# XingqunQi-lab/EmotionGestures

Hardware: AMD Instinct MI355X
Metric: gesture clips/sec (34 frames, 43 joints) (higher is better)
Workload: dtype bf16x3; 1 GPU; TED clips: 4 s 16 kHz audio -> mel(128x124) -> CVAE sample -> generator -> 34x126 pose; global_batch=64, variant=Models_spatial_memory, parallelism=clip-sharded x1, no data-path collective, launch=hipGraph replay, 4 step(s) in flight, branch_streams=False, fold_affine=False

## Files before the change

### emotiongestures_amd/_lib.py

```python
from __future__ import annotations

import ctypes as C
import os

_HERE = os.path.dirname(os.path.abspath(__file__))
LIB_PATH = os.path.join(_HERE, "libemogest_hip.so")

EG_PREC_F32, EG_PREC_BF16X3, EG_PREC_BF16 = 0, 1, 2
PRECISIONS = {"f32": EG_PREC_F32, "fp32": EG_PREC_F32, "bf16x3": EG_PREC_BF16X3, "bf16": EG_PREC_BF16}

(PACK_RAW, PACK_LINEAR, PACK_VEC_PAD, PACK_CONV3X3, PACK_BN_SCALE, PACK_BN_SHIFT, PACK_CONV1X1, PACK_STEM,
 PACK_WN_TAP, PACK_CONV1D, PACK_POS_TABLE, PACK_LINEAR_T, PACK_LINEAR_FOLD, PACK_BIAS_FOLD, PACK_CONV1X1_BF16, PACK_WN_TAPS) = range(16)


class EgError(RuntimeError):
    pass


class EgWeightEntry(C.Structure):
    _fields_ = [("key", C.c_char * 192), ("kind", C.c_int32), ("dims", C.c_int32 * 4),
                ("offset", C.c_int64), ("numel", C.c_int64)]


class EgGeneratorConfig(C.Structure):
# ... 52 lines not shown
    "eg_generator_forward_rollout": (C.c_int, [_P, _P, _I, _I, _P, _P, _P, _P, _P, _P, _P, _P, _P, _P, _P, _P, _L, _P]),
    "eg_generator_rollout_workspace_bytes": (_L, [_P, _I, _I]),
    "eg_generator_forward_rollout_draws": (C.c_int, [_P, _P, _I, _I, _I, _P, _P, _P, _P, _P, _P, _P, _P, _P, _P, _P, _P, _L, _P]),
    "eg_generator_rollout_draws_workspace_bytes": (_L, [_P, _I, _I, _I]),
    "eg_rows_by_table": (C.c_int, [_P, _P, _P, _I, _L, _I, _P]),
    "eg_rollout_ragged_plan_ints": (_L, [_I, _L]),
    "eg_rollout_ragged_plan": (C.c_int, [_P, _I, _P, _P, _P, _P]),
    "eg_generator_forward_rollout_ragged": (C.c_int, [_P, _P, _I, _P, _P, _P, _P, _P, _P, _P, _P, _P, _P, _P, _P, _P, _P, _L, _P]),
    "eg_generator_rollout_ragged_workspace_bytes": (_L, [_P, _I, _L]),
    "eg_rollout_takes_plan_ints": (_L, [_I, _L]),
    "eg_rollout_takes_plan": (C.c_int, [_P, _I, _P, _P, _P, _P]),
    "eg_generator_forward_rollout_takes": (C.c_int, [_P, _P, _I, _I, _P, _P, _P, _P, _P, _P, _P, _P, _P, _P, _P, _P, _P, _P, _L, _P]),
    "eg_generator_rollout_takes_workspace_bytes": (_L, [_P, _I, _L, _I]),
    "eg_stream_state_bytes": (_L, [_P, _I, _I, _I]),
    "eg_stream_reset": (C.c_int, [_P, _P, _I, _I, _I, _P, _P, _P]),
    "eg_stream_push": (C.c_int, [_P, _P, _I, _I, _I, _P, _P, _P, _P]),
    "eg_generator_stream_step": (C.c_int, [_P, _P, _P, _I, _I, _I, _P, _P, _P, _P, _P, _P, _P, _P, _P, _L, _P]),
    "eg_stream_tail": (C.c_int, [_P, _P, _I, _I, _I, _P, _P]),
    "eg_generator_tap": (C.c_int, [_P, _I, _P, C.c_char_p, C.POINTER(_P), C.POINTER(_L)]),
    "eg_cvae_default_config": (C.c_int, [C.POINTER(EgCvaeConfig)]),
    "eg_cvae_create": (C.c_int, [C.POINTER(EgCvaeConfig), C.POINTER(_P)]),
    "eg_cvae_destroy": (None, [_P]),
    "eg_cvae_arena_floats": (_L, [_P]),
    "eg_cvae_num_weights": (_I, [_P]),
    "eg_cvae_weight_entry": (C.c_int, [_P, _I, C.POINTER(EgWeightEntry)]),
    "eg_cvae_workspace_bytes": (_L, [_P, _I]),
    "eg_cvae_sample": (C.c_int, [_P, _P, _I, _P, _P, _P, _P, _L, _P]),
    "eg_cvae_forward": (C.c_int, [_P, _P, _I, _P, _P, _P, _P, _P, _P, _P, _L, _P]),
    "eg_mel_tables": (C.c_int, [_P, _P, _P, _P]),
    "eg_mel_workspace_bytes": (_L, [_I, _I]),
    "eg_melspectrogram": (C.c_int, [_P, _I, _I, _P, _P, _P, _P, _P, _I, _P, _L, _P]),
    "eg_window_gather": (C.c_int, [_P, _I, _L, _I, _L, _I, _P, _P]),
    "eg_window_gather_ragged": (C.c_int, [_P, _I, _L, _P, _P, _L, _I, _P, _P]),
    "eg_resample_plan": (C.c_int, [_I, _I, C.POINTER(EgResamplePlan)]),
    "eg_resample_out_length": (_L, [_L, _I, _I]),
    "eg_resample_filter": (C.c_int, [_I, _I, _P, _P]),
    "eg_resample": (C.c_int, [_P, _I, _L, _P, _P, _I, _I, _P, _L, _P, _L, _P]),
    "eg_resample_stream_state_bytes": (_L, [_I, _I, _I]),
    "eg_resample_stream_reset": (C.c_int, [_P, _I, _I, _I, _P, _P]),
    "eg_resample_stream_push": (C.c_int, [_P, _I, _I, _I, _P, _P, _I, _P, _P, _I, _P]),
    "eg_skeleton_check": (C.c_int, [_P, _P, _P, _I]),
    "eg_skeleton_out_frames": (_L, [_L, _I, _I]),
    "eg_skeleton_tile_frames": (_I, []),
    "eg_skeleton_joints": (C.c_int, [_P, _I, _I, _P, _P, _P, _I, _P, _P, _I, _I, _P, _I, _I, _I, _P, _L, _P]),
    "eg_skeleton_dir_vec": (C.c_int, [_P, _I, _I, _P, _P, _P, _I, _P, _P, _I, _I, _P, _P, _P]),
    "eg_skeleton_rest_check": (C.c_int, [_P, _I]),
    "eg_skeleton_levels": (C.c_int, [_P, _P, _P, _I, _P, _P]),
    "eg_skeleton_rotations": (C.c_int, [_P, _I, _I, _P, _P, _P, _I, _P, _P, _P, _I, _I, _P, _I, _I, _I, _P, _L, _P]),
    "eg_articulate_check": (C.c_int, [_P, _P, _I]),
    "eg_articulate_levels": (C.c_int, [_P, _P, _I, _P]),
    "eg_articulate_tile_frames": (_I, []),
    "eg_articulate_forward": (C.c_int, [_P, _I, _I, _P, _P, _I, _P, _P, _I, _I, _P, _I, _I, _I, _I, _P, _P, _L, _P]),
    "eg_articulate_rot6d": (C.c_int, [_P, _I, _I, _I, _P, _I, _I, _P, _I, _P, _P]),
    "eg_articulate_euler": (C.c_int, [_P, _I, _I, _I, _P, _P, _P, _I, _I, _P, _I, _I, _I, _I, _P, _L, _P]),
    "eg_articulate_rot6d_euler": (C.c_int, [_P, _I, _I, _I, _P, _P, _P, _I, _I, _P, _I, _I, _P, _P]),
    "eg_angle_unwrap_workspace_bytes": (_L, [_I, _I, _I]),
    "eg_angle_unwrap": (C.c_int, [_P, _I, _I, _I, _P, _I, _I, C.c_double, _P, _L, _P]),
    "eg_smooth_design": (C.c_int, [_I, _I, _I, C.c_double, _P, _P]),
    "eg_smooth_tile_frames": (_I, []),
    "eg_smooth_tile_cols": (_I, []),
    "eg_smooth_tracks": (C.c_int, [_P, _I, _I, _I, _I, _P, _P, _P, _I, _I, _P, _P]),
    "eg_smooth_stream_state_bytes": (_L, [_I, _I, _I]),
    "eg_smooth_stream_reset": (C.c_int, [_P, _I, _I, _I, _P, _P]),
    "eg_smooth_stream_push": (C.c_int, [_P, _I, _I, _I, _I, _P, _P, _P, _P, _P]),
    "eg_smooth_stream_tail": (C.c_int, [_P, _I, _I, _I, _I, _P, _P, _P, _P]),
    "eg_beat_tables": (C.c_int, [_P, _P, _P, _P]),
    "eg_beat_workspace_bytes": (_L, [_I, _I]),
    "eg_beat_align": (C.c_int, [_P, _I, _I, _P, _I, _I, _I, _I, _I, C.c_double, _I, _P, _P, _P, _P, _P, _L, _P, _P, _P, _P, _P, _P, _P]),
    "eg_beat_tracks_meta_ints": (_L, [_I]),
    "eg_beat_tracks_meta": (C.c_int, [_P, _P, _P, _I, _I, _P]),
    "eg_beat_tracks_workspace_bytes": (_L, [_P, _P, _I, _I, _I]),
    "eg_beat_align_tracks": (C.c_int, [_P, _I, _L, _P, _P, _P, _I, _I, _I, _P, _I, _I, _P, C.c_double, _I, _P, _P, _P, _P, _P, _L, _P, _P, _P,
                                       _P, _P, _P, _P]),
    "eg_beat_tracks_scan": (C.c_int, [_P, _P, _I, _P, _P, _L, _P, _P, _P]),
    "eg_take_meta_ints": (_L, [_I]),
    "eg_take_meta": (C.c_int, [_P, _I, _P]),
    "eg_track_rows_pack": (C.c_int, [_P, _I, _I, _I, _I, _P, _P, _P, _P]),
    "eg_take_distance_workspace_bytes": (_L, [_P, _I, _I]),
    "eg_take_distance": (C.c_int, [_P, _I, _I, _I, _P, _P, _I, _P, _L, _P, _P, _P]),
    "eg_conv3x3": (C.c_int, [_P, _P, _P, _P, _P, _P, _P, _I, _I, _I, _I, _I, _I, _I, _I, _I, _P]),
    "eg_conv3x3_se": (C.c_int, [_P, _P, _P, _P, _P, _P, _P, _P, _P, _I, _I, _I, _I, _I, _I, _I, _I, _I, _P]),
    "eg_se_gate_pre": (C.c_int, [_P, _P, _I, _P, _P, _P, _P, _P, _P, _P, _P, _I, _I, _I, _I, _P]),
    "eg_se_block_fused": (C.c_int, [_P] * 19 + [_I] * 7 + [_P]),
    "eg_conv3x3_gap_tiles": (_I, [_I, _I, _I, _I, _I]),
    "eg_conv3x3_channel_split": (_I, [_I, _I, _I, _I, _I, _I, _I]),
    "eg_stem_conv": (C.c_int, [_P, _P, _P, _P, _P, _P, _I, _I, _I, _I, _P]),
    "eg_se_gate": (C.c_int, [_P, _I, _P, _P, _P, _P, _P, _I, _I, _I, _P]),
    "eg_se_residual_relu": (C.c_int, [_P, _P, _P, _P, _P, _P, _P, _I, _I, _I, _I, _I, _I, _I, _I, _P]),
    "eg_linear": (C.c_int, [_P, _I, _P, _I, _P, _P, _P, _I, _P, _I, _I, _I, _I, _I, _I, _I, _I, _P]),
    "eg_split_tiles": (C.c_int, [_P, _I, _I, _I, _P, _P]),
    "eg_linear_presplit": (C.c_int, [_P, _I, _P, _I, _P, _P, _P, _I, _P, _I, _I, _I, _I, _I, _I, _P]),
    "eg_linear_presplit_causal": (C.c_int, [_P, _I, _P, _P, _I, _P, _P, _I, _P, _I, _P, _I, _I, _I, _I, _I, _I, _I, _I, _P]),
    "eg_linear_splitk": (C.c_int, [_P, _I, _P, _I, _P, _P, _I, _I, _I, _I, _I, _I, _P, _I, _P]),
    "eg_layernorm": (C.c_int, [_P, _P, _P, _P, _I, _I, C.c_float, _P]),
    "eg_attention": (C.c_int, [_P, _I, _P, _I, _P, _I, _P, _I, _P, _I, _I, _I, _I, _I, _I, _P]),
    "eg_attention_masked": (C.c_int, [_P, _I, _P, _I, _P, _I, _P, _L, _I, _P, _I, _P, _I, _I, _I, _I, _I, _I, _P]),
    "eg_mha_workspace_bytes": (_L, [_I, _I, _I, _I, _I]),
    "eg_multi_head_attention": (C.c_int, [_P, _P, _P, _P, _P, _P, _P, _P, _P, _P, _I, _I, _I, _I, _I, _I, _P, _L, _P]),
    "eg_ffn_workspace_bytes": (_L, [_I, _I, _I]),
    "eg_positionwise_ffn": (C.c_int, [_P, _P, _P, _P, _P, _P, _P, _P, _I, _I, _I, _I, _P, _L, _P]),
    "eg_tcn_forward": (C.c_int, [_P, _P, _P, _I, _I, _I, _I, _I, _P, _L, _P]),
    "eg_add_rows": (C.c_int, [_P, _P, _P, _L, _I, _I, _P]),
    "eg_add_rows_split": (C.c_int, [_P, _P, _P, _P, _L, _I, _I, _P]),
    "eg_conv3x3_packed_floats": (_L, [_I, _I]),
    "eg_profile_enable": (C.c_int, [_I]),
    "eg_profile_disable": (C.c_int, []),
    "eg_profile_read": (_I, [_P, _P, _P, _I]),
    "eg_profile_read_workgroups": (_I, [_P, _I]),
    "eg_time_linear": (C.c_int, [_P, _P, _P, _P, _I, _I, _I, _I, _P]),
    "eg_reparameterize": (C.c_int, [_P, _P, _P, _P, _L, _P]),
    "eg_conv1d": (C.c_int, [_P, _P, _P, _P, _P, _P, _I, _I, _I, _I, _I, _I, _I, _I, _P]),
    "eg_contrastive_workspace_bytes": (C.c_int64, [_I]),
    "eg_contrastive_loss": (C.c_int, [_P, _P, _I, _I, _P, _P, _P, _P, _L, _P]),
    "eg_contrastive_backward_workspace_bytes": (_L, [_I]),
    "eg_contrastive_loss_backward": (C.c_int, [_P, _P, _I, _I, _P, _P, _P, _L, _P]),
    "eg_transpose": (C.c_int, [_P, _I, _I, _I, _P, _I, _P]),
    "eg_gemm_tn_workspace_floats": (_L, [_I, _I, _L]),
    "eg_gemm_tn": (C.c_int, [_P, _I, _P, _I, _P, _I, _I, _I, _L, _P, _L, _I, _P]),
    "eg_conv3x3_wgrad": (C.c_int, [_P, _P, _P, _I, _I, _I, _I, _I, _I, _P, _L, _P]),
    "eg_im2col3x3": (C.c_int, [_P, _P, _I, _I, _I, _I, _I, _I, _P]),
    "eg_subsample": (C.c_int, [_P, _P, _I, _I, _I, _I, _I, _I, _P]),
    "eg_conv1d_cl_forward": (C.c_int, [_P, _P, _P, _P] + [_I] * 9 + [_P]),
    "eg_conv1d_cl_backward_input": (C.c_int, [_P, _P, _P, _P] + [_I] * 9 + [_P]),
    "eg_conv1d_cl_backward_weight_workspace_floats": (_L, [_I] * 7),
    "eg_conv1d_cl_backward_weight": (C.c_int, [_P, _P, _P, _P, _P] + [_I] * 9 + [_P, _L, _P]),
    "eg_pad_cols": (C.c_int, [_P, _P, _L, _I, _I, _P]),
    "eg_colreduce_workspace_floats": (_L, [_I]),
    "eg_bn_train_forward": (C.c_int, [_P, _P, _P, _P, _P, _P, _P, _P, _L, _I, C.c_float, C.c_float, _P, _P]),
    "eg_bn_train_backward": (C.c_int, [_P, _P, _P, _P, _P, _P, _P, _P, _L, _I, _I, _P, _P]),
    "eg_bn_train_forward_gap": (C.c_int, [_P, _P, _I, _I, _P, _P, _P, _P, _P, _P, _P, _P, _L, _I, C.c_float, C.c_float, _P, _P]),
    "eg_bn_train_forward_sq": (C.c_int, [_P, _P, _P, _I, _I, _P, _P, _P, _P, _P, _P, _P, _P, _L, _I, C.c_float, C.c_float, _P, _P]),
    "eg_conv3x3_sq": (C.c_int, [_P, _P, _P, _P, _P, _P] + [_I] * 8 + [_P]),
    "eg_se_gate_train_forward": (C.c_int, [_P] * 12 + [_I, _I, _I, _P]),
    "eg_se_tail_forward": (C.c_int, [_P] * 9 + [_I, _I, _I, _P]),
    "eg_se_tail_backward_reduce": (C.c_int, [_P] * 7 + [_I, _I, _I, _P, _P]),
    "eg_se_gate_train_backward": (C.c_int, [_P] * 16 + [_I, _I, _I, _P]),
    "eg_se_tail_backward_finish": (C.c_int, [_P] * 14 + [_I, _I, _I, _P]),
    "eg_se_tail_backward_apply": (C.c_int, [_P] * 13 + [_I, _I, _I, _P]),
    "eg_colsum": (C.c_int, [_P, _P, _P, _P, _L, _I, _P, _P]),
    "eg_elementwise": (C.c_int, [_P, _P, _P, _L, _I, C.c_float, _P]),
    "eg_conv3x3_wgrad_mfma_workspace_floats": (_L, [_I, _I, _I, _I, _I]),
    "eg_conv3x3_wgrad_mfma": (C.c_int, [_P, _P, _P, _I, _I, _I, _I, _I, _P, _L, _P]),
    "eg_conv3x3_wgrad_mfma_oihw": (C.c_int, [_P, _P, _P, _I, _I, _I, _I, _I, _P, _L, _P]),
    "eg_conv3x3_wgrad_gather_mfma": (C.c_int, [_P, _P, _P, _I, _I, _I, _I, _I, _I, _P, _L, _P]),
    "eg_conv3x3_dgrad_s2": (C.c_int, [_P, _P, _P, _P, _I, _I, _I, _I, _I, _I, _P]),
    "eg_conv3x3_res_masked": (C.c_int, [_P, _P, _P, _P, _P, _I, _I, _I, _I, _I, _I, _P]),
    "eg_conv3x3_wgrad_mfma_oihw_in_affine": (C.c_int, [_P, _P, _P, _P, _P, _I, _I, _I, _I, _I, _P, _L, _P]),
    "eg_conv3x3_sq_in_affine": (C.c_int, [_P, _P, _P, _P, _P, _P, _P, _P, _I, _I, _I, _I, _I, _I, _I, _I, _P]),
    "eg_bn_train_stats_sq": (C.c_int, [_P, _P, _I, _I, _P, _P, _P, _P, _P, _P, _P, _P, _L, _I, C.c_float, C.c_float, _P, _P]),
    "eg_pack_conv3x3_device": (C.c_int, [_P, _I, _I, _I, _P, _P]),
    "eg_linear_packed_floats": (_L, [_I, _I]),
    "eg_pack_linear_device": (C.c_int, [_P, _I, _I, _I, _I, _P, _P]),
    "eg_pack_table_blocks": (_I, [_I, _I, _I, _I]),
    "eg_pack_table": (C.c_int, [_P, _I, _I, _P]),
    "eg_dropout": (C.c_int, [_P, _P, _L, C.c_float, C.c_uint32, C.c_uint64, _P]),
    "eg_dropout_dev": (C.c_int, [_P, _P, _L, C.c_float, C.c_uint32, C.c_uint64, _P, _P]),
    "eg_seg_mean": (C.c_int, [_P, _P, _I, _I, _I, C.c_float, _P, _P]),
    "eg_seg_dot": (C.c_int, [_P, _P, _P, _I, _I, _I, _P, _P]),
    "eg_se_scale": (C.c_int, [_P, _P, _P, _P, _I, _I, _I, _P]),
    "eg_layernorm_backward": (C.c_int, [_P, _P, _P, _P, _P, _I, _I, C.c_float, _P]),
    "eg_attention_train": (C.c_int, [_P, _I, _P, _I, _P, _I, _P, _I, _P, _I, _I, _I, _I, _I, C.c_float, C.c_uint32, C.c_uint64, _P, _P]),
    "eg_attention_backward_train": (C.c_int, [_P, _I, _P, _I, _P, _I, _P, _P, _I, _P, _I, _P, _I, _P, _I, _I, _I, _I, _I, _I, C.c_float, C.c_uint32,
                                              C.c_uint64, _P, _P]),
    "eg_smooth_l1": (C.c_int, [_P, _P, _P, _P, _L, C.c_float, C.c_float, _P, _P]),
    "eg_cross_entropy": (C.c_int, [_P, _P, _P, C.c_float, C.c_float, _P, _P, _I, _I, _P, _P]),
    "eg_kld": (C.c_int, [_P, _P, _P, _P, _P, _I, _I, C.c_float, _P]),
# ... 53 lines not shown
```

### emotiongestures_amd/csrc/conv.hip

```cpp
#include <type_traits>
#include "common.h"


namespace {

struct ConvArgs {
    const float* x; const float* w; const float* bias; const float* scale; const float* shift;
    float* y; float* gap;
    float* gap2 = nullptr;
    int H, W, Ho, Wo, cout, relu, nchw, tiles_x, tiles;
    const float* gate = nullptr; const float* res = nullptr; int relu2 = 0;
    const float* in_scale = nullptr; const float* in_shift = nullptr;
    int wrow = 0;
    const unsigned* res_bits = nullptr;
    const float* res_q = nullptr;
    unsigned int* dbg = nullptr;
    const float* sc_x = nullptr; const bf8* sc_whi = nullptr; const bf8* sc_wlo = nullptr; const float* sc_vec = nullptr;
    int sc_H = 0, sc_W = 0, sc_S = 2, sc_B = 0;
};
__device__ __forceinline__ f4 residual_quad(const float* __restrict__ res, const unsigned* __restrict__ bits, size_t e) {
    f4 r = *reinterpret_cast<const f4*>(res + e);
    if (bits) {
        const unsigned nb = bits[e >> 5] >> (unsigned)(e & 28);
        r[0] = (nb & 1u) ? r[0] : 0.f;
        r[1] = (nb & 2u) ? r[1] : 0.f;
        r[2] = (nb & 4u) ? r[2] : 0.f;
        r[3] = (nb & 8u) ? r[3] : 0.f;
    }
    return r;
}

template <int S, int TH> struct ConvGeom {
    static constexpr int IH = (TH - 1) * S + 3;
    static constexpr int IW = 31 * S + 3;
    static constexpr int NPIX = IH * IW;
    static constexpr int PL = (S == 1) ? ((NPIX + 15) / 16 * 16) : (NPIX | 1);
    static constexpr int MT = TH * 2 / 4;
};

template <int TH> struct ConvGeomDG2 {
    static constexpr int IH = TH + 1;
    static constexpr int IW = 33;
    static constexpr int NPIX = IH * IW;
    static constexpr int PL = (NPIX + 15) / 16 * 16;
};

template <int CIN, int NT, int S, int TH>
__global__ __launch_bounds__(256) void conv3x3_f32_kernel(ConvArgs a) {
    using G = ConvGeom<S, TH>;
    constexpr int COUTP = NT * 16, IW = G::IW, NPIX = G::NPIX, PL = G::PL, MT = G::MT;
    __shared__ f4 tile[8 * PL];

    const int tid = threadIdx.x, wave = tid >> 6, lane = tid & 63, li = lane & 15, kq = lane >> 4;
    int tile_id = blockIdx.x, b = blockIdx.y;
    {
        const int total = gridDim.x * gridDim.y;
        if ((total & 7) == 0) {
            const int lin = blockIdx.y * gridDim.x + blockIdx.x;
            const int log = (lin & 7) * (total >> 3) + (lin >> 3);
            b = log / (int)gridDim.x;
            tile_id = log - b * (int)gridDim.x;
        }
    }
    const int ty = tile_id / a.tiles_x, tx = tile_id - ty * a.tiles_x;
    const int oy0 = ty * TH, ox0 = tx * 32;
    const int iy0 = oy0 * S - 1, ix0 = ox0 * S - 1;

    int pbase[MT];
#pragma unroll
    for (int t = 0; t < MT; ++t) {
        const int id = wave * MT + t;
        pbase[t] = ((id >> 1) * S) * IW + ((id & 1) * 16 + li) * S;
    }
    f4 acc[MT][NT];
#pragma unroll
    for (int t = 0; t < MT; ++t)
#pragma unroll
        for (int n = 0; n < NT; ++n) acc[t][n] = (f4){0.f, 0.f, 0.f, 0.f};

    const f4* __restrict__ w4 = reinterpret_cast<const f4*>(a.w);
    const float* __restrict__ xb = a.x + (size_t)b * a.H * a.W * CIN;

    for (int chunk = 0; chunk < CIN / 32; ++chunk) {
        if (chunk) __syncthreads();
        for (int idx = tid; idx < ((NPIX + 7) / 8) * 64; idx += 256) {
            const int p = (idx >> 6) * 8 + (idx & 7), cq = (idx >> 3) & 7;
            if (p < NPIX) {
                const int iy = p / IW, ix = p - iy * IW;
                const int gy = iy0 + iy, gx = ix0 + ix;
                f4 v = (f4){0.f, 0.f, 0.f, 0.f};
                if (gy >= 0 && gy < a.H && gx >= 0 && gx < a.W)
                    v = *reinterpret_cast<const f4*>(xb + ((size_t)gy * a.W + gx) * CIN + chunk * 32 + cq * 4);
                tile[cq * PL + p] = v;
            }
        }
        __syncthreads();
        const f4* wp = w4 + (size_t)(chunk * 8 + kq) * COUTP + li;
#pragma unroll 1
        for (int kh = 0; kh < 3; ++kh) {
#pragma unroll
            for (int kw = 0; kw < 3; ++kw) {
                const int tap = kh * 3 + kw, toff = kh * IW + kw;
// ... 393 lines not shown
    for (int t = 0; t < MT; ++t) {
        const int id = wm * MT + t;
        const int oy = oy0 + (id >> 1), ox = ox0 + (id & 1) * 16 + li;
        pixo[t] = (oy < a.Ho && ox < a.Wo) ? oy * a.Wo + ox : -1;
    }
    const int hw = a.Ho * a.Wo;
    float* __restrict__ yb = a.y + (size_t)b * hw * a.cout;
#pragma unroll
    for (int n = 0; n < NT; ++n) {
        gsum[n] = (f4){0.f, 0.f, 0.f, 0.f};
        gsq[n] = gsum[n];
        const int co = c0 + (wn * NT + n) * 16 + kq * 4;
        const f4 bi = a.bias ? *reinterpret_cast<const f4*>(a.bias + co) : (f4){0.f, 0.f, 0.f, 0.f};
        f4 sc = a.scale ? *reinterpret_cast<const f4*>(a.scale + co) : (f4){1.f, 1.f, 1.f, 1.f};
        f4 sh = a.shift ? *reinterpret_cast<const f4*>(a.shift + co) : (f4){0.f, 0.f, 0.f, 0.f};
        if constexpr (SCC > 0) {
            const float* __restrict__ qv = a.sc_vec + ((size_t)a.sc_B + b) * a.cout + co;
            sc = *reinterpret_cast<const f4*>(qv);
            sh = *reinterpret_cast<const f4*>(qv + (size_t)a.sc_B * a.cout);
        }
        const f4 gt = (a.gate && co < a.cout) ? *reinterpret_cast<const f4*>(a.gate + (size_t)b * a.cout + co) : (f4){1.f, 1.f, 1.f, 1.f};
        const bool rb = a.res != nullptr;
        const size_t rbase = (size_t)b * hw * a.cout;
#pragma unroll
        for (int t = 0; t < MT; ++t) {
            f4 v = acc[0][t][n] + bi;
            if (a.relu) {
#pragma unroll
                for (int r = 0; r < 4; ++r) v[r] = fmaxf(v[r], 0.f);
            }
            v = v * sc + sh;
            if (a.gate) v = v * gt;
            if (rb && pixo[t] >= 0 && co < a.cout) v += residual_quad(a.res, a.res_bits, rbase + (size_t)pixo[t] * a.cout + co);
            if (a.relu2) {
#pragma unroll
                for (int r = 0; r < 4; ++r) v[r] = fmaxf(v[r], 0.f);
            }
            if (pixo[t] >= 0) {
                if (!a.nchw) {
                    if (co < a.cout) *reinterpret_cast<f4*>(yb + pixo[t] * a.cout + co) = v;
                } else {
#pragma unroll
                    for (int r = 0; r < 4; ++r)
                        if (co + r < a.cout) yb[(co + r) * hw + pixo[t]] = v[r];
                }
                gsum[n] += v;
                if (a.gap2) gsq[n] += v * v;
            }
        }
    }
    if (a.gap) {
        float* sred = reinterpret_cast<float*>(lds);
#pragma unroll
        for (int n = 0; n < NT; ++n) {
#pragma unroll
            for (int r = 0; r < 4; ++r) {
                float s = gsum[n][r];
                s = row16_sum(s);
                if (li == 0) sred[wm * COUTP + (wn * NT + n) * 16 + kq * 4 + r] = s;
                if (a.gap2) {
                    float q = gsq[n][r];
                    q = row16_sum(q);
                    if (li == 0) sred[(WM + wm) * COUTP + (wn * NT + n) * 16 + kq * 4 + r] = q;
                }
            }
        }
        wait_lgkmcnt0();
        wg_barrier();
        if (tid < (SPLIT ? COUTP : a.cout)) {
            float s = 0.f;
#pragma unroll
            for (int m = 0; m < WM; ++m) s += sred[m * COUTP + tid];
            a.gap[((size_t)b * a.tiles + tile_id) * a.cout + c0 + tid] = s;
            if (a.gap2) {
                float q = 0.f;
#pragma unroll
                for (int m = 0; m < WM; ++m) q += sred[(WM + m) * COUTP + tid];
                a.gap2[((size_t)b * a.tiles + tile_id) * a.cout + c0 + tid] = q;
            }
        }
    }
}

template <int TERMS, int TH = 4, bool STAMP = false>
__global__ __launch_bounds__(256, 2) void conv3x3_c32_persistent_kernel(ConvArgs a, const bf8* __restrict__ whi, const bf8* __restrict__ wlo,
                                                                     int total_tiles, int tiles_per_wg) {
    using G = ConvGeom<1, TH>;
    constexpr int CIN = 32, IW = G::IW, NPIX = G::NPIX, PL = G::PL, MT = TH / 2, NT = 2;
    constexpr int NIMG = (TERMS == 3) ? 2 : 1;
    constexpr int TILE = NIMG * 4 * PL, WTAP = 4 * 32, WIMG = 9 * WTAP;
    static_assert(PL - NPIX >= 8 || TH == 4, "the gap scratch of the 8-row variant lives in the planes' padding slots");
    extern __shared__ __attribute__((aligned(16))) bf8 lds[];
    bf8* tile = lds;
    bf8* wl = lds + TILE;
    float* sred_base = reinterpret_cast<float*>(lds + TILE + NIMG * WIMG);
    const int sred_pitch = (TH == 4) ? 32 : PL * 4;
    float* sred = (TH == 4) ? sred_base : reinterpret_cast<float*>(tile + NPIX);

    const int tid = threadIdx.x, wave = tid >> 6, lane = tid & 63, li = lane & 15, kq = lane >> 4;
    const int wave_u = __builtin_amdgcn_readfirstlane(wave);
    int wg = blockIdx.x;
    if ((gridDim.x & 7) == 0) wg = (blockIdx.x & 7) * (gridDim.x >> 3) + (blockIdx.x >> 3);
    const int NWG = gridDim.x;
    const int t_begin = wg, t_end = total_tiles;
    (void)tiles_per_wg;
    if (t_begin >= t_end) return;

#pragma unroll
    for (int img = 0; img < NIMG; ++img) {
        const bf8* src = img ? wlo : whi;
#pragma unroll
        for (int p = 0; p < 5; ++p) {
            const int piece = p * 4 + wave_u;
            if (piece < WIMG / 64)
                __builtin_amdgcn_global_load_lds((const __attribute__((address_space(1))) void*)(src + piece * 64 + lane),
                                                 (__attribute__((address_space(3))) void*)(wl + img * WIMG + piece * 64), 16, 0, 0);
        }
    }

    constexpr int NIT = (((NPIX + 7) / 8) * 32 + 255) / 256;
    int piy[NIT], pix[NIT], lslot[NIT];
#pragma unroll
    for (int it = 0; it < NIT; ++it) {
        const int idx = tid + it * 256;
        const int p = (idx >> 5) * 8 + (idx & 7), oc = (idx >> 3) & 3;
        piy[it] = p / IW;
        pix[it] = p - piy[it] * IW;
        lslot[it] = p < NPIX ? oc * PL + p : -1;
    }
    const int oc8 = ((tid >> 3) & 3) * 8;
    f4 isc[2] = {(f4){1.f, 1.f, 1.f, 1.f}, (f4){1.f, 1.f, 1.f, 1.f}}, ish[2] = {(f4){0.f, 0.f, 0.f, 0.f}, (f4){0.f, 0.f, 0.f, 0.f}};
    if (a.in_scale) {
        isc[0] = *reinterpret_cast<const f4*>(a.in_scale + oc8); isc[1] = *reinterpret_cast<const f4*>(a.in_scale + oc8 + 4);
        ish[0] = *reinterpret_cast<const f4*>(a.in_shift + oc8); ish[1] = *reinterpret_cast<const f4*>(a.in_shift + oc8 + 4);
    }
    f4 pv[NIT][2];
    struct Coord { int b, ty, tx; };
    const int tiles_y = a.tiles / a.tiles_x;
    const int adv_b = NWG / a.tiles, adv_r = NWG - adv_b * a.tiles, adv_ty = adv_r / a.tiles_x, adv_tx = adv_r - adv_ty * a.tiles_x;
    auto advance = [&](Coord& c) {
        c.tx += adv_tx;
        if (c.tx >= a.tiles_x) { c.tx -= a.tiles_x; ++c.ty; }
        c.ty += adv_ty;
        if (c.ty >= tiles_y) { c.ty -= tiles_y; ++c.b; }
        c.b += adv_b;
    };
    auto load_tile = [&](const Coord& c) {
        const int b = c.b;
        const int iy0 = c.ty * TH - 1, ix0 = c.tx * 32 - 1;
        const float* __restrict__ xb = a.x + (size_t)b * a.H * a.W * CIN;
#pragma unroll
        for (int it = 0; it < NIT; ++it) {
            pv[it][0] = pv[it][1] = (f4){0.f, 0.f, 0.f, 0.f};
            const int gy = iy0 + piy[it], gx = ix0 + pix[it];
            if (lslot[it] >= 0 && gy >= 0 && gy < a.H && gx >= 0 && gx < a.W) {
                const float* src = xb + (gy * a.W + gx) * CIN + oc8;
                pv[it][0] = *reinterpret_cast<const f4*>(src);
                pv[it][1] = *reinterpret_cast<const f4*>(src + 4);
                if (a.in_scale) {
                    pv[it][0] = pv[it][0] * isc[0] + ish[0];
                    pv[it][1] = pv[it][1] * isc[1] + ish[1];
                }
            }
        }
    };
    auto store_tile = [&]() {
#pragma unroll
        for (int it = 0; it < NIT; ++it) {
            if (lslot[it] >= 0) {
                bf8 hi, lo;
                split_octet<TERMS == 3>(pv[it][0], pv[it][1], hi, lo);
                tile[lslot[it]] = hi;
                if (TERMS == 3) tile[4 * PL + lslot[it]] = lo;
            }
        }
    };
    int pbase[MT];
#pragma unroll
    for (int t = 0; t < MT; ++t) {
        const int id = wave * MT + t;
        pbase[t] = (id >> 1) * IW + (id & 1) * 16 + li;
    }
    struct Frags { bf8 wh[NT], wlf[NT], xh[MT], xl[MT]; };
    auto read_frags = [&](Frags& f, int tap) {
        const bf8* Wh = wl + tap * WTAP + kq * 32 + li;
        const int kh = tap / 3, kw = tap - kh * 3, toff = kh * IW + kw;
#pragma unroll
        for (int n = 0; n < NT; ++n) {
            f.wh[n] = Wh[n * 16];
            if (TERMS == 3) f.wlf[n] = Wh[WIMG + n * 16];
        }
#pragma unroll
        for (int t = 0; t < MT; ++t) {
            f.xh[t] = tile[kq * PL + pbase[t] + toff];
            if (TERMS == 3) f.xl[t] = tile[(4 + kq) * PL + pbase[t] + toff];
        }
    };

    const int hw = a.Ho * a.Wo;
    f4 bi[NT], sc[NT], sh[NT];
#pragma unroll
    for (int n = 0; n < NT; ++n) {
        const int co = n * 16 + kq * 4;
        bi[n] = a.bias ? *reinterpret_cast<const f4*>(a.bias + co) : (f4){0.f, 0.f, 0.f, 0.f};
        sc[n] = a.scale ? *reinterpret_cast<const f4*>(a.scale + co) : (f4){1.f, 1.f, 1.f, 1.f};
        sh[n] = a.shift ? *reinterpret_cast<const f4*>(a.shift + co) : (f4){0.f, 0.f, 0.f, 0.f};
    }

    f4 rsn[MT][NT];
    auto load_res = [&](const Coord& c) {
        const int ty = c.ty, tx = c.tx;
        const size_t rbase = (size_t)c.b * hw * 32;
#pragma unroll
        for (int t = 0; t < MT; ++t) {
            const int id = wave * MT + t;
            const int oy = ty * TH + (id >> 1), ox = tx * 32 + (id & 1) * 16 + li;
            const bool ok = a.res && oy < a.Ho && ox < a.Wo;
#pragma unroll
            for (int n = 0; n < NT; ++n)
                rsn[t][n] = ok ? residual_quad(a.res, a.res_bits, rbase + (size_t)(oy * a.Wo + ox) * 32 + n * 16 + kq * 4) : (f4){0.f, 0.f, 0.f, 0.f};
        }
    };
    Coord cur;
    cur.b = t_begin / a.tiles;
    cur.ty = (t_begin - cur.b * a.tiles) / a.tiles_x;
    cur.tx = t_begin - cur.b * a.tiles - cur.ty * a.tiles_x;
    Coord nxt = cur;
    load_tile(cur);
    load_res(cur);
    wait_vmcnt_imm<0>();
    unsigned int ph[6] = {0, 0, 0, 0, 0, 0};
    unsigned long long tk = 0;
    auto stamp = [&](int i) {
        if constexpr (STAMP) {
            const unsigned long long now = __builtin_amdgcn_s_memtime();
            if (i >= 0) ph[i] += (unsigned int)(now - tk);
            tk = now;
        }
    };
    for (int L = t_begin; L < t_end; L += NWG, cur = nxt) {
        const int b = cur.b, tile_id = cur.ty * a.tiles_x + cur.tx;
        const int oy0 = cur.ty * TH, ox0 = cur.tx * 32;
        advance(nxt);
        stamp(-1);
        store_tile();
        stamp(0);
        __syncthreads();
        stamp(1);
        int pixo[MT];
        f4 rs[MT][NT];
#pragma unroll
        for (int t = 0; t < MT; ++t) {
            const int id = wave * MT + t;
            const int oy = oy0 + (id >> 1), ox = ox0 + (id & 1) * 16 + li;
            pixo[t] = (oy < a.Ho && ox < a.Wo) ? oy * a.Wo + ox : -1;
#pragma unroll
            for (int n = 0; n < NT; ++n) rs[t][n] = rsn[t][n];
        }
        const bool has_res = a.res != nullptr;
        if (L + NWG < t_end) load_res(nxt);
        if (L + NWG < t_end) load_tile(nxt);
        stamp(2);

        f4 acc[MT][NT];
#pragma unroll
        for (int t = 0; t < MT; ++t)
#pragma unroll
            for (int n = 0; n < NT; ++n) acc[t][n] = (f4){0.f, 0.f, 0.f, 0.f};
        Frags fr[2];
        read_frags(fr[0], 0);
#pragma unroll
        for (int tap = 0; tap < 9; ++tap) {
            if (tap < 8) read_frags(fr[(tap + 1) & 1], tap + 1);
            const Frags& f = fr[tap & 1];
#pragma unroll
            for (int t = 0; t < MT; ++t)
#pragma unroll
                for (int n = 0; n < NT; ++n) {
                    if (TERMS == 3) {
                        acc[t][n] = __builtin_amdgcn_mfma_f32_16x16x32_bf16(f.wlf[n], f.xh[t], acc[t][n], 0, 0, 0);
                        acc[t][n] = __builtin_amdgcn_mfma_f32_16x16x32_bf16(f.wh[n], f.xl[t], acc[t][n], 0, 0, 0);
                    }
                    acc[t][n] = __builtin_amdgcn_mfma_f32_16x16x32_bf16(f.wh[n], f.xh[t], acc[t][n], 0, 0, 0);
                }
        }

        if constexpr (STAMP) {
#pragma unroll
            for (int t = 0; t < MT; ++t)
#pragma unroll
                for (int n = 0; n < NT; ++n) asm volatile("" : "+v"(acc[t][n]));
        }
        stamp(3);
        float* __restrict__ yb = a.y + (size_t)b * hw * 32;
        f4 gsum[NT], gsq[NT];
#pragma unroll
        for (int n = 0; n < NT; ++n) {
            gsum[n] = (f4){0.f, 0.f, 0.f, 0.f};
            gsq[n] = gsum[n];
            const int co = n * 16 + kq * 4;
            const f4 gt = a.gate ? *reinterpret_cast<const f4*>(a.gate + (size_t)b * 32 + co) : (f4){1.f, 1.f, 1.f, 1.f};
#pragma unroll
            for (int t = 0; t < MT; ++t) {
                f4 v = acc[t][n] + bi[n];
                if (a.relu) {
#pragma unroll
                    for (int r = 0; r < 4; ++r) v[r] = fmaxf(v[r], 0.f);
                }
                v = v * sc[n] + sh[n];
                if (a.gate) v = v * gt;
                if (has_res && pixo[t] >= 0) v += rs[t][n];
                if (a.relu2) {
#pragma unroll
                    for (int r = 0; r < 4; ++r) v[r] = fmaxf(v[r], 0.f);
                }
                if (pixo[t] >= 0) {
                    *reinterpret_cast<f4*>(yb + pixo[t] * 32 + co) = v;
                    gsum[n] += v;
                    if (a.gap2) gsq[n] += v * v;
                }
            }
        }
        if (a.gap) {
#pragma unroll
            for (int n = 0; n < NT; ++n)
#pragma unroll
                for (int r = 0; r < 4; ++r) {
                    float sm = gsum[n][r];
                    sm = row16_sum(sm);
                    if (li == 0) sred[wave * sred_pitch + n * 16 + kq * 4 + r] = sm;
                    if (a.gap2) {
                        float q = gsq[n][r];
                        q = row16_sum(q);
                        if (li == 0) sred[128 + wave * 32 + n * 16 + kq * 4 + r] = q;
                    }
                }
        }
        stamp(4);
        __syncthreads();
        stamp(5);
        if (a.gap && tid < 32) {
            float sm = 0.f;
#pragma unroll
            for (int m = 0; m < 4; ++m) sm += sred[m * sred_pitch + tid];
            a.gap[((size_t)b * a.tiles + tile_id) * 32 + tid] = sm;
            if (a.gap2) a.gap2[((size_t)b * a.tiles + tile_id) * 32 + tid] = (sred[128 + tid] + sred[160 + tid]) + (sred[192 + tid] + sred[224 + tid]);
        }
    }
    if constexpr (STAMP) {
        if (lane == 0 && a.dbg)
#pragma unroll
            for (int i = 0; i < 6; ++i) a.dbg[((size_t)blockIdx.x * 4 + wave) * 8 + i] = ph[i];
    }
}

__global__ __launch_bounds__(256) void stem_conv_kernel(const float* __restrict__ x, const float* __restrict__ w,
                                                        const float* __restrict__ bias, const float* __restrict__ scale,
                                                        const float* __restrict__ shift, float* __restrict__ y,
                                                        int B, int H, int W, int C) {
    extern __shared__ float rows[];
    const int cq_n = C >> 2, tid = threadIdx.x;
    const int b = blockIdx.x / H, oy = blockIdx.x - b * H, WP = W + 2;
    const float* xb = x + (size_t)b * H * W;
    for (int i = tid; i < 3 * WP; i += 256) {
        const int r = i / WP, c = i - r * WP, gy = oy + r - 1, gx = c - 1;
        rows[i] = (gy >= 0 && gy < H && gx >= 0 && gx < W) ? xb[gy * W + gx] : 0.f;
    }
    const int cq = tid % cq_n, px0 = tid / cq_n, pstep = 256 / cq_n;
    f4 wv[9];
#pragma unroll
    for (int t = 0; t < 9; ++t) wv[t] = *reinterpret_cast<const f4*>(w + t * C + cq * 4);
    const f4 bi = *reinterpret_cast<const f4*>(bias + cq * 4);
    const f4 sc = *reinterpret_cast<const f4*>(scale + cq * 4), sh = *reinterpret_cast<const f4*>(shift + cq * 4);
    __syncthreads();
    float* yrow = y + ((size_t)b * H + oy) * W * C + cq * 4;
    for (int ox = px0; ox < W; ox += pstep) {
        f4 acc = bi;
#pragma unroll
        for (int kh = 0; kh < 3; ++kh)
#pragma unroll
            for (int kw = 0; kw < 3; ++kw) acc += wv[kh * 3 + kw] * rows[kh * WP + ox + kw];
#pragma unroll
        for (int r = 0; r < 4; ++r) acc[r] = fmaxf(acc[r], 0.f);
        *reinterpret_cast<f4*>(yrow + (size_t)ox * C) = acc * sc + sh;
    }
}

__global__ __launch_bounds__(256) void se_gate_kernel(const float* __restrict__ gap, int tiles, const float* __restrict__ w1,
                                                      const float* __restrict__ b1, const float* __restrict__ w2,
                                                      const float* __restrict__ b2, float* __restrict__ gate, int C, float inv_hw) {
    __shared__ float m[256];
    __shared__ float h[32];
    const int b = blockIdx.x, t = threadIdx.x, R = C >> 3;
    {
        const int c = t % C, g = t / C, G = blockDim.x / C;
        float s = 0.f;
        for (int i = g; i < tiles; i += G) s += gap[((size_t)b * tiles + i) * C + c];
        m[t] = s;
        __syncthreads();
        float tot = 0.f;
        if (t < C)
            for (int j = 0; j < G; ++j) tot += m[j * C + t];
        __syncthreads();
        if (t < C) m[t] = tot * inv_hw;
    }
    __syncthreads();
    if (t < R) {
        float s = b1[t];
        for (int c = 0; c < C; ++c) s += w1[t * C + c] * m[c];
        h[t] = fmaxf(s, 0.f);
    }
    __syncthreads();
    if (t < C) {
        float s = b2[t];
        for (int j = 0; j < R; ++j) s += w2[t * R + j] * h[j];
        gate[(size_t)b * C + t] = 1.f / (1.f + expf(-s));
    }
}

constexpr int GP_T = 1024;
__global__ __launch_bounds__(GP_T) void se_gate_pre_kernel(const float* __restrict__ t1, const float* __restrict__ gap, int tiles,
                                                           const float* __restrict__ w2img, const float* __restrict__ scale2,
                                                           const float* __restrict__ shift2, const float* __restrict__ w1, const float* __restrict__ b1,
                                                           const float* __restrict__ wf2, const float* __restrict__ bf2, float* __restrict__ gate,
                                                           int H, int W, int C, const float* __restrict__ ds_scale, const float* __restrict__ ds_shift,
                                                           float* __restrict__ sc_vec) {
    extern __shared__ __attribute__((aligned(16))) float sm[];
    const int b = blockIdx.x, t = threadIdx.x, G = GP_T / C, c = t % C, g = t / C, R = C >> 3;
    float* part = sm;
    float* S = sm + 5 * GP_T;
    float* zp = S + 9 * C;
    float* m = zp + GP_T;
    float* hbuf = m + C;
    const float* tb = t1 + (size_t)b * H * W * C;
    float s0 = 0.f, s1 = 0.f, s2 = 0.f, s3 = 0.f, s4 = 0.f;
#pragma unroll 4
    for (int i = g; i < tiles; i += G) s0 += gap[((size_t)b * tiles + i) * C + c];
#pragma unroll 4
    for (int x = g; x < W; x += G) {
        s1 += tb[(size_t)x * C + c];
        s2 += tb[((size_t)(H - 1) * W + x) * C + c];
    }
#pragma unroll 4
    for (int y = g; y < H; y += G) {
        s3 += tb[((size_t)y * W) * C + c];
        s4 += tb[((size_t)y * W + W - 1) * C + c];
    }
    part[t] = s0; part[GP_T + t] = s1; part[2 * GP_T + t] = s2; part[3 * GP_T + t] = s3; part[4 * GP_T + t] = s4;
    __syncthreads();
    if (t < C) {
        float T = 0.f, R0 = 0.f, RL = 0.f, C0 = 0.f, CL = 0.f;
        for (int j = 0; j < G; ++j) {
            T += part[j * C + t]; R0 += part[GP_T + j * C + t]; RL += part[2 * GP_T + j * C + t]; C0 += part[3 * GP_T + j * C + t];
            CL += part[4 * GP_T + j * C + t];
        }
        const float c00 = tb[t], c0L = tb[(size_t)(W - 1) * C + t], cL0 = tb[((size_t)(H - 1) * W) * C + t], cLL = tb[((size_t)(H - 1) * W + W - 1) * C + t];
#pragma unroll
        for (int kh = 0; kh < 3; ++kh)
#pragma unroll
            for (int kw = 0; kw < 3; ++kw) {
                const float rex = kh == 0 ? RL : (kh == 2 ? R0 : 0.f);
                const float cex = kw == 0 ? CL : (kw == 2 ? C0 : 0.f);
                float corner = 0.f;
                if (kh == 0 && kw == 0) corner = cLL;
                if (kh == 0 && kw == 2) corner = cL0;
                if (kh == 2 && kw == 0) corner = c0L;
                if (kh == 2 && kw == 2) corner = c00;
// ... 86 lines not shown
        }
        const f4 res = acc * *reinterpret_cast<const f4*>(dss + cq * 4) + *reinterpret_cast<const f4*>(dsh + cq * 4);
        const f4 g = *reinterpret_cast<const f4*>(gate + (size_t)b * COUT + cq * 4);
        f4 v = *reinterpret_cast<const f4*>(y + p * COUT + cq * 4) * g + res;
#pragma unroll
        for (int r = 0; r < 4; ++r) v[r] = fmaxf(v[r], 0.f);
        *reinterpret_cast<f4*>(out + p * COUT + cq * 4) = v;
      }
    }
}

template <int CIN, int NT, int S, int TH, int WM, int WN, int TERMS, int SCC = 0>
int launch_conv_bf16(const ConvArgs& a, const bf8* whi, const bf8* wlo, dim3 grid, hipStream_t st) {
    constexpr int RING = 3;
    using G = ConvGeom<S, TH>;
    constexpr int NIMG = (TERMS == 3) ? 2 : 1;
    constexpr size_t LDS_BYTES = sizeof(bf8) * (size_t)(NIMG * 4 * G::PL + RING * NIMG * 4 * NT * 16);
    auto kern = conv3x3_bf16_kernel<CIN, NT, S, TH, WM, WN, TERMS, RING, false, false, SCC>;
    if (int rc = eg_ensure_dynamic_lds(reinterpret_cast<const void*>(kern), LDS_BYTES, "conv3x3")) return rc;
    hipLaunchKernelGGL(kern, grid, dim3(256), LDS_BYTES, st, a, whi, wlo);
    return eg_check_launch("conv3x3");
}

template <int CIN, int NTS, int TH, int WM, int WN, int TERMS, int SCC = 0>
int launch_conv_split_t(ConvArgs a, int batch, const bf8* whi, const bf8* wlo, hipStream_t st) {
    constexpr int RING = 3;
    using G = ConvGeom<1, TH>;
    constexpr int NIMG = (TERMS == 3) ? 2 : 1;
    constexpr size_t LDS_BYTES = sizeof(bf8) * (size_t)(NIMG * 4 * G::PL + RING * NIMG * 4 * NTS * 16);
    auto kern = conv3x3_bf16_kernel<CIN, NTS, 1, TH, WM, WN, TERMS, RING, true, false, SCC>;
    if (int rc = eg_ensure_dynamic_lds(reinterpret_cast<const void*>(kern), LDS_BYTES, "conv3x3 (channel split)")) return rc;
    a.wrow = a.cout;
    hipLaunchKernelGGL(kern, dim3(a.tiles, batch, a.cout / (NTS * 16)), dim3(256), LDS_BYTES, st, a, whi, wlo);
    return eg_check_launch("conv3x3 (channel split)");
}
template <int KCH, int NTN, int TH, int WM, int WN>
int launch_dgrad_s2_t(const ConvArgs& a, int batch, const bf8* whi, const bf8* wlo, hipStream_t st) {
    constexpr int RING = 3;
    using G = ConvGeomDG2<TH>;
    constexpr size_t LDS_BYTES = sizeof(bf8) * (size_t)(2 * 4 * G::PL + RING * 2 * 4 * NTN * 16);
    auto kern = conv3x3_bf16_kernel<KCH, NTN, 1, TH, WM, WN, 3, RING, false, true>;
    if (int rc = eg_ensure_dynamic_lds(reinterpret_cast<const void*>(kern), LDS_BYTES, "conv3x3 (stride-2 input gradient)")) return rc;
    dim3 grid(eg_cdiv(a.W, 32) * eg_cdiv(a.H, TH), batch);
    hipLaunchKernelGGL(kern, grid, dim3(256), LDS_BYTES, st, a, whi, wlo);
    return eg_check_launch("conv3x3 (stride-2 input gradient)");
}
int conv_channel_split(int wgs, int max_split) {
    const char* e = getenv("EG_CONV_SPLIT");
    const int forced = (e && e[0]) ? atoi(e) : -1;
    if (forced >= 0) return (forced == 2 || forced == 4) && forced <= max_split ? forced : 1;
    int split = 1;
    while (split < max_split && wgs * split * 2 <= 512) split *= 2;
    return split;
}

int body_channel_split(int batch, int tiles, int cin, int cout, int stride, int precision, int nchw_out) {
    if (!((cin == 64 || cin == 128) && cout == cin && stride == 1 && precision == EG_PREC_BF16X3 && !nchw_out)) return 1;
    return conv_channel_split(tiles * batch, cin == 128 ? 4 : 2);
}

template <int CIN, int NT, int S, int TH, int WM, int WN, int SCC = 0>
int launch_conv(const ConvArgs& a, int batch, int precision, hipStream_t st) {
    dim3 grid(a.tiles, batch), block(256);
    if (precision == EG_PREC_F32) {
        if constexpr (SCC > 0) {
            eg_set_error("conv3x3: the fused downsample shortcut exists in the split-bf16 modes only");
            return EG_ERR_UNSUPPORTED;
        }
        hipLaunchKernelGGL((conv3x3_f32_kernel<CIN, NT, S, TH>), grid, block, 0, st, a);
        return eg_check_launch("conv3x3");
    }
    const size_t f32_floats = (size_t)9 * CIN * NT * 16;
    const bf8* whi = reinterpret_cast<const bf8*>(a.w + f32_floats);
    const bf8* wlo = whi + (size_t)9 * (CIN / 8) * NT * 16;
    if (precision == EG_PREC_BF16X3) return launch_conv_bf16<CIN, NT, S, TH, WM, WN, 3, SCC>(a, whi, wlo, grid, st);
    return launch_conv_bf16<CIN, NT, S, TH, WM, WN, 1, SCC>(a, whi, wlo, grid, st);
}

bool conv32_persistent_enabled() {
    static const bool on = [] { const char* e = getenv("EG_CONV32_PERSISTENT"); return !(e && e[0] == '0'); }();
    return on;
}

template <int TERMS, int TH>
int launch_conv32_persistent_t(const ConvArgs& a, int batch, const bf8* whi, const bf8* wlo, hipStream_t st) {
    using G = ConvGeom<1, TH>;
    constexpr int NIMG = (TERMS == 3) ? 2 : 1;
    constexpr size_t LDS_BYTES = sizeof(bf8) * (size_t)(NIMG * 4 * G::PL + NIMG * 9 * 128) + (TH == 4 ? 2 * 4 * 32 * sizeof(float) : 0);
    auto kern = conv3x3_c32_persistent_kernel<TERMS, TH>;
    if (int rc = eg_ensure_dynamic_lds(reinterpret_cast<const void*>(kern), LDS_BYTES, "conv3x3 (32 -> 32, persistent)")) return rc;
    const int total = a.tiles * batch;
    const int cap = 512;
    int grid = total < cap ? total : cap;
    int tpw = eg_cdiv(total, grid);
    grid = eg_cdiv(total, tpw);
    if (grid >= 8) grid = (int)eg_round_up(grid, 8);
    hipLaunchKernelGGL(kern, dim3(grid), dim3(256), LDS_BYTES, st, a, whi, wlo, total, tpw);
    return eg_check_launch("conv3x3 (32 -> 32, persistent)");
}
int launch_conv32_persistent(const ConvArgs& a, int batch, int precision, int th, hipStream_t st) {
    const size_t f32_floats = (size_t)9 * 32 * 32;
    const bf8* whi = reinterpret_cast<const bf8*>(a.w + f32_floats);
    const bf8* wlo = whi + (size_t)9 * 4 * 32;
    static const bool stamp = [] { const char* e = getenv("EG_CONV32_STAMP"); return e && e[0] == '1'; }();
    if (stamp && precision == EG_PREC_BF16X3 && th == 4) {
        static unsigned int* dbg = nullptr;
        const int nwords = 512 * 4 * 8;
        if (!dbg && hipMalloc(&dbg, nwords * sizeof(unsigned int)) != hipSuccess) return EG_ERR_HIP;
        (void)hipMemsetAsync(dbg, 0, nwords * sizeof(unsigned int), st);
        ConvArgs b = a;
        b.dbg = dbg;
        constexpr size_t LDS_BYTES = sizeof(bf8) * (size_t)(2 * 4 * ConvGeom<1, 4>::PL + 2 * 9 * 128) + 2 * 4 * 32 * sizeof(float);
        auto kern = conv3x3_c32_persistent_kernel<3, 4, true>;
        if (int rc = eg_ensure_dynamic_lds(reinterpret_cast<const void*>(kern), LDS_BYTES, "conv3x3 (stamps)")) return rc;
        const int total = a.tiles * batch;
        int grid = total < 512 ? total : 512;
        grid = eg_cdiv(total, eg_cdiv(total, grid));
        if (grid >= 8) grid = (int)eg_round_up(grid, 8);
        hipLaunchKernelGGL(kern, dim3(grid), dim3(256), LDS_BYTES, st, b, whi, wlo, total, 0);
        static unsigned int host[512 * 4 * 8];
        if (hipMemcpyAsync(host, dbg, sizeof(host), hipMemcpyDeviceToHost, st) != hipSuccess || hipStreamSynchronize(st) != hipSuccess) return EG_ERR_HIP;
        double sum[6] = {0, 0, 0, 0, 0, 0};
        int nw = 0;
        for (int w = 0; w < grid * 4; ++w) {
            if (host[w * 8 + 3] == 0) continue;
            ++nw;
            for (int i = 0; i < 6; ++i) sum[i] += host[w * 8 + i];
        }
        const double tiles_per_wave = (double)total / grid;
        fprintf(stderr, "conv32 stamps (cycles per tile and wave, %d waves, %s residual): store_tile %.0f  barrier1 %.0f  issue_loads %.0f  taps %.0f  epilogue %.0f  barrier2 %.0f\n",
                nw, a.res ? "with" : "no", sum[0] / nw / tiles_per_wave, sum[1] / nw / tiles_per_wave, sum[2] / nw / tiles_per_wave, sum[3] / nw / tiles_per_wave,
                sum[4] / nw / tiles_per_wave, sum[5] / nw / tiles_per_wave);
        return eg_check_launch("conv3x3 (32 -> 32, stamps)");
    }
    if (th == 8) {
        if (precision == EG_PREC_BF16X3) return launch_conv32_persistent_t<3, 8>(a, batch, whi, wlo, st);
        return launch_conv32_persistent_t<1, 8>(a, batch, whi, wlo, st);
    }
    if (precision == EG_PREC_BF16X3) return launch_conv32_persistent_t<3, 4>(a, batch, whi, wlo, st);
    return launch_conv32_persistent_t<1, 4>(a, batch, whi, wlo, st);
}

int conv_tile_rows(int cin, int cout, int stride) {
    if (stride == 2 || cout >= 256) return 2;
    if (cin == 32 && cout == 32) {
        static const int th = [] { const char* e = getenv("EG_CONV32_TH"); return (e && atoi(e) == 8) ? 8 : 4; }();
        return th;
    }
    return (cout >= 128 || cin >= 128) ? 4 : 8;
}

}

extern "C" int32_t eg_conv3x3_gap_tiles(int32_t h, int32_t wdt, int32_t cin, int32_t cout, int32_t stride) {
    const int ho = (h + 2 - 3) / stride + 1, wo = (wdt + 2 - 3) / stride + 1;
    const int th = conv_tile_rows(cin, cout, stride);
    return eg_cdiv(ho, th) * eg_cdiv(wo, 32);
}

extern "C" int32_t eg_conv3x3_channel_split(int32_t batch, int32_t h, int32_t wdt, int32_t cin, int32_t cout, int32_t stride, int32_t precision) {
    return body_channel_split(batch, eg_conv3x3_gap_tiles(h, wdt, cin, cout, stride), cin, cout, stride, precision, 0);
}

extern "C" int64_t eg_conv3x3_packed_floats(int32_t cin, int32_t cout_pad) {
    return (int64_t)9 * cin * cout_pad * 2;
}

extern "C" int eg_conv3x3(const float* x, const float* w, const float* bias, const float* scale, const float* shift,
                          float* y, float* gap_partial, int32_t batch, int32_t h, int32_t wdt, int32_t cin, int32_t cout,
                          int32_t stride, int32_t relu, int32_t nchw_out, int32_t precision, void* stream) {
    return eg_conv3x3_se(x, w, bias, scale, shift, nullptr, nullptr, y, gap_partial, batch, h, wdt, cin, cout, stride, relu, nchw_out, precision, stream);
}

namespace {
struct ShortcutArgs { const float* x; const float* wimg; const float* vec; int h, w, cin, stride; };
int conv3x3_dispatch(const float* x, const float* w, const float* bias, const float* scale, const float* shift, const float* gate, const float* residual,
                     float* y, float* gap_partial, float* gap_sq, int32_t batch, int32_t h, int32_t wdt, int32_t cin, int32_t cout, int32_t stride,
                     int32_t relu, int32_t nchw_out, int32_t precision, void* stream, const float* in_scale = nullptr, const float* in_shift = nullptr,
                     const uint32_t* res_bits = nullptr, const ShortcutArgs* sc = nullptr);
}
extern "C" int eg_conv3x3_se(const float* x, const float* w, const float* bias, const float* scale, const float* shift, const float* gate,
                             const float* residual, float* y, float* gap_partial, int32_t batch, int32_t h, int32_t wdt, int32_t cin,
                             int32_t cout, int32_t stride, int32_t relu, int32_t nchw_out, int32_t precision, void* stream) {
    return conv3x3_dispatch(x, w, bias, scale, shift, gate, residual, y, gap_partial, nullptr, batch, h, wdt, cin, cout, stride, relu, nchw_out, precision, stream);
}
extern "C" int eg_conv3x3_res_masked(const float* x, const float* w, const float* residual, const uint32_t* res_bits, float* y, int32_t batch, int32_t h,
                                     int32_t wdt, int32_t cin, int32_t cout, int32_t precision, void* stream) {
    EG_REQUIRE(residual && res_bits, EG_ERR_BAD_ARG, "eg_conv3x3_res_masked: the residual and its bit mask are required");
    return conv3x3_dispatch(x, w, nullptr, nullptr, nullptr, nullptr, residual, y, nullptr, nullptr, batch, h, wdt, cin, cout, 1, 0, 0, precision, stream, nullptr,
                            nullptr, res_bits);
}
extern "C" int eg_conv3x3_sq(const float* x, const float* w, const float* bias, float* y, float* gap_partial, float* gap_sq_partial, int32_t batch, int32_t h,
                             int32_t wdt, int32_t cin, int32_t cout, int32_t stride, int32_t relu, int32_t precision, void* stream) {
    EG_REQUIRE(gap_partial && gap_sq_partial, EG_ERR_BAD_ARG, "eg_conv3x3_sq: both partial buffers are required");
    EG_REQUIRE(precision != EG_PREC_F32, EG_ERR_UNSUPPORTED, "eg_conv3x3_sq: split-bf16 modes only (the fp32 kernel emits sums only)");
    EG_REQUIRE(!(cin == 32 && cout == 32 && stride == 1) || conv_tile_rows(cin, cout, stride) == 4, EG_ERR_UNSUPPORTED,
               "eg_conv3x3_sq: the 8-row experiment tiles of the 32 -> 32 kernel have no room for the squares scratch");
    return conv3x3_dispatch(x, w, bias, nullptr, nullptr, nullptr, nullptr, y, gap_partial, gap_sq_partial, batch, h, wdt, cin, cout, stride, relu, 0, precision,
                            stream);
}
extern "C" int eg_conv3x3_sq_in_affine(const float* x, const float* in_scale, const float* in_shift, const float* w, const float* bias, float* y,
                                       float* gap_partial, float* gap_sq_partial, int32_t batch, int32_t h, int32_t wdt, int32_t cin, int32_t cout,
                                       int32_t stride, int32_t relu, int32_t precision, void* stream) {
    EG_REQUIRE(in_scale && in_shift, EG_ERR_BAD_ARG, "eg_conv3x3_sq_in_affine: both affine vectors are required");
    EG_REQUIRE(!gap_partial == !gap_sq_partial, EG_ERR_BAD_ARG, "eg_conv3x3_sq_in_affine: both partial buffers or none");
    return conv3x3_dispatch(x, w, bias, nullptr, nullptr, nullptr, nullptr, y, gap_partial, gap_sq_partial, batch, h, wdt, cin, cout, stride, relu, 0, precision,
                            stream, in_scale, in_shift);
}
namespace {
int conv3x3_dispatch(const float* x, const float* w, const float* bias, const float* scale, const float* shift, const float* gate, const float* residual,
                     float* y, float* gap_partial, float* gap_sq, int32_t batch, int32_t h, int32_t wdt, int32_t cin, int32_t cout, int32_t stride,
                     int32_t relu, int32_t nchw_out, int32_t precision, void* stream, const float* in_scale, const float* in_shift, const uint32_t* res_bits,
                     const ShortcutArgs* sc) {
    EG_REQUIRE(x && w && y && batch > 0 && h > 0 && wdt > 0, EG_ERR_BAD_ARG, "eg_conv3x3: null pointer or empty shape");
    EG_REQUIRE(!res_bits || (residual && !gate && ((size_t)batch * h * wdt * cout) % 32 == 0), EG_ERR_BAD_ARG,
               "eg_conv3x3_res_masked: the bit mask needs a residual, no gate and a map of a multiple of 32 elements");
    EG_REQUIRE((in_scale == nullptr) == (in_shift == nullptr) && (!in_scale || (precision != EG_PREC_F32 && cin % 32 == 0 && eg_aligned16(in_scale) &&
               eg_aligned16(in_shift))), EG_ERR_BAD_ARG, "eg_conv3x3: the input affine needs both vectors, a split-bf16 mode and cin %% 32 == 0");
    EG_REQUIRE(!gate || residual, EG_ERR_BAD_ARG, "eg_conv3x3_se: a gate needs a residual");
    EG_REQUIRE(!residual || (!nchw_out && stride == 1 && cout % 4 == 0 && (!gate || eg_aligned16(gate)) && eg_aligned16(residual) && residual != y),
               EG_ERR_BAD_ARG, "eg_conv3x3_se: the fused residual needs NHWC output, stride 1, cout %% 4 == 0 and a residual buffer distinct from y");
    EG_REQUIRE(eg_aligned16(x) && eg_aligned16(w) && eg_aligned16(y), EG_ERR_ALIGN, "eg_conv3x3: pointers must be 16-byte aligned");
    EG_REQUIRE(stride == 1 || stride == 2, EG_ERR_UNSUPPORTED, "eg_conv3x3: stride %d", stride);
    EG_REQUIRE(precision >= 0 && precision <= 2, EG_ERR_BAD_ARG, "eg_conv3x3: precision %d", precision);
    EG_REQUIRE(nchw_out || (cout % 4 == 0), EG_ERR_UNSUPPORTED, "eg_conv3x3: NHWC output needs cout %% 4 == 0");
    ConvArgs a;
    a.x = x; a.w = w; a.bias = bias; a.scale = scale; a.shift = shift; a.y = y; a.gap = gap_partial; a.gap2 = gap_sq;
    a.gate = gate; a.res = residual; a.relu2 = gate ? 1 : 0;
    a.res_bits = res_bits;
    a.in_scale = in_scale; a.in_shift = in_shift;
    a.H = h; a.W = wdt; a.Ho = (h + 2 - 3) / stride + 1; a.Wo = (wdt + 2 - 3) / stride + 1;
    a.cout = cout; a.relu = relu; a.nchw = nchw_out;
    const int th = conv_tile_rows(cin, cout, stride);
    a.tiles_x = eg_cdiv(a.Wo, 32);
    a.tiles = a.tiles_x * eg_cdiv(a.Ho, th);
    hipStream_t st = (hipStream_t)stream;
    const int coutp = (int)eg_round_up(cout, 16);
    EgProfScope prof((int64_t)cin * 1000000 + (int64_t)cout * 1000 + stride * 100 + 1,
                     2.0 * 9 * cin * cout * (double)a.Ho * a.Wo * batch, st);
    if (sc) {
        EG_REQUIRE(precision != EG_PREC_F32 && stride == 1 && !nchw_out && cout == cin && (cin == 64 || cin == 128) && sc->cin * 2 == cin, EG_ERR_UNSUPPORTED,
                   "conv3x3: the fused downsample shortcut serves 32 -> 64 and 64 -> 128 block entries in the split-bf16 modes (cin=%d cout=%d shortcut cin=%d)",
                   cin, cout, sc->cin);
        EG_REQUIRE(sc->x && sc->wimg && sc->vec && !gate && !residual && !bias && !relu && !gap_sq && !in_scale && sc->stride >= 1 &&
                   (sc->h - 1) / sc->stride + 1 == h && (sc->w - 1) / sc->stride + 1 == wdt && eg_aligned16(sc->x) && eg_aligned16(sc->wimg) &&
                   eg_aligned16(sc->vec), EG_ERR_BAD_ARG, "conv3x3: fused downsample shortcut: null / misaligned operand or a block input that does not map onto the output");
        a.sc_x = sc->x; a.sc_vec = sc->vec; a.sc_H = sc->h; a.sc_W = sc->w; a.sc_S = sc->stride; a.sc_B = batch;
        a.sc_whi = reinterpret_cast<const bf8*>(sc->wimg);
        a.sc_wlo = a.sc_whi + (size_t)(sc->cin / 8) * cout;
        a.scale = a.shift = nullptr;
        a.relu2 = 1;
        const int split = body_channel_split(batch, a.tiles, cin, cout, 1, precision, 0);
        const bf8* whi = reinterpret_cast<const bf8*>(a.w + (size_t)9 * cin * cout);
        const bf8* wlo = whi + (size_t)9 * (cin / 8) * cout;
        if (cin == 64 && split == 2) return launch_conv_split_t<64, 2, 8, 4, 1, 3, 1>(a, batch, whi, wlo, st);
        if (cin == 64) return launch_conv<64, 4, 1, 8, 4, 1, 1>(a, batch, precision, st);
        if (split == 2) return launch_conv_split_t<128, 4, 4, 2, 2, 3, 2>(a, batch, whi, wlo, st);
        if (split == 4) return launch_conv_split_t<128, 2, 4, 2, 2, 3, 2>(a, batch, whi, wlo, st);
        return launch_conv<128, 8, 1, 4, 2, 2, 2>(a, batch, precision, st);
    }
    if (cin == 32 && coutp == 32 && cout == 32 && stride == 1 && precision != EG_PREC_F32 && !nchw_out && conv32_persistent_enabled())
        return launch_conv32_persistent(a, batch, precision, th, st);
    if (cin == 32 && coutp == 32 && stride == 1 && th == 4) return launch_conv<32, 2, 1, 4, 4, 1>(a, batch, precision, st);
    if (cin == 32 && coutp == 32 && stride == 1) return launch_conv<32, 2, 1, 8, 4, 1>(a, batch, precision, st);
    if (cin == 32 && coutp == 64 && stride == 2) return launch_conv<32, 4, 2, 2, 2, 2>(a, batch, precision, st);
    if (const int split = body_channel_split(batch, a.tiles, cin, cout, stride, precision, nchw_out); split > 1) {
        const size_t f32_floats = (size_t)9 * cin * cout;
        const bf8* whi = reinterpret_cast<const bf8*>(a.w + f32_floats);
        const bf8* wlo = whi + (size_t)9 * (cin / 8) * cout;
        if (cin == 64 && split == 2) return launch_conv_split_t<64, 2, 8, 4, 1, 3>(a, batch, whi, wlo, st);
        if (cin == 128 && split == 2) return launch_conv_split_t<128, 4, 4, 2, 2, 3>(a, batch, whi, wlo, st);
        if (cin == 128 && split == 4) return launch_conv_split_t<128, 2, 4, 2, 2, 3>(a, batch, whi, wlo, st);
    }
    if (cin == 64 && coutp == 64 && stride == 1) return launch_conv<64, 4, 1, 8, 4, 1>(a, batch, precision, st);
    if (cin == 64 && coutp == 128 && stride == 2) return launch_conv<64, 8, 2, 2, 2, 2>(a, batch, precision, st);
    if (cin == 64 && coutp == 128 && stride == 1) return launch_conv<64, 8, 1, 4, 2, 2>(a, batch, precision, st);
    if (cin == 128 && coutp == 128 && stride == 1) return launch_conv<128, 8, 1, 4, 2, 2>(a, batch, precision, st);
    if (cin == 128 && coutp == 256 && stride == 2) return launch_conv<128, 16, 2, 2, 1, 4>(a, batch, precision, st);
    if (cin == 256 && coutp == 256 && stride == 1) return launch_conv<256, 16, 1, 2, 1, 4>(a, batch, precision, st);
    if (cin == 128 && coutp <= 64 && stride == 1) {
        if (coutp <= 48) return launch_conv<128, 3, 1, 4, 4, 1>(a, batch, precision, st);
        return launch_conv<128, 4, 1, 4, 4, 1>(a, batch, precision, st);
    }
    if (cin == 128 && coutp <= 128 && stride == 1) return launch_conv<128, 8, 1, 4, 2, 2>(a, batch, precision, st);
    eg_set_error("eg_conv3x3: unsupported channels cin=%d cout=%d stride=%d", cin, cout, stride);
    return EG_ERR_UNSUPPORTED;
}
}

extern "C" int eg_conv3x3_dgrad_s2(const float* dy, const float* w_flip, const float* res_q, float* dx, int32_t batch, int32_t h, int32_t wdt, int32_t cin,
                                   int32_t cout, int32_t precision, void* stream) {
    EG_REQUIRE(dy && w_flip && dx && batch > 0 && h > 0 && wdt > 0, EG_ERR_BAD_ARG, "eg_conv3x3_dgrad_s2: null pointer or empty shape");
    EG_REQUIRE(precision == EG_PREC_BF16X3, EG_ERR_UNSUPPORTED, "eg_conv3x3_dgrad_s2: split-bf16 arithmetic only (precision %d)", precision);
    EG_REQUIRE(eg_aligned16(dy) && eg_aligned16(w_flip) && eg_aligned16(dx) && (!res_q || eg_aligned16(res_q)), EG_ERR_ALIGN,
               "eg_conv3x3_dgrad_s2: pointers must be 16-byte aligned");
    ConvArgs a;
    a.x = dy; a.w = w_flip; a.bias = nullptr; a.scale = nullptr; a.shift = nullptr; a.y = dx; a.gap = nullptr;
    a.H = (h - 1) / 2 + 1; a.W = (wdt - 1) / 2 + 1; a.Ho = h; a.Wo = wdt;
    a.cout = cin; a.relu = 0; a.nchw = 0; a.tiles_x = eg_cdiv(a.W, 32); a.tiles = 0;
    a.res_q = res_q;
    hipStream_t st = (hipStream_t)stream;
    const size_t f32_floats = (size_t)9 * cout * cin;
    const bf8* whi = reinterpret_cast<const bf8*>(w_flip + f32_floats);
    const bf8* wlo = whi + (size_t)9 * (cout / 8) * cin;
    EgProfScope prof((int64_t)cin * 1000000 + (int64_t)cout * 1000 + 200 + 8, 2.0 * 9 * cin * cout * (double)a.H * a.W * batch, st);
    if (cin == 32 && cout == 64) return launch_dgrad_s2_t<64, 2, 4, 4, 1>(a, batch, whi, wlo, st);
    if (cin == 64 && cout == 128) return launch_dgrad_s2_t<128, 4, 2, 2, 2>(a, batch, whi, wlo, st);
    if (cin == 128 && cout == 256) return launch_dgrad_s2_t<256, 8, 1, 1, 4>(a, batch, whi, wlo, st);
    eg_set_error("eg_conv3x3_dgrad_s2: unsupported channels %d -> %d", cin, cout);
    return EG_ERR_UNSUPPORTED;
}

extern "C" int eg_stem_conv(const float* x, const float* w9xc, const float* bias, const float* scale, const float* shift,
                            float* y, int32_t batch, int32_t h, int32_t wdt, int32_t c, void* stream) {
    EG_REQUIRE(x && w9xc && bias && scale && shift && y && batch > 0, EG_ERR_BAD_ARG, "eg_stem_conv: null pointer");
    EG_REQUIRE(c % 4 == 0 && c <= 128 && 256 % (c / 4) == 0, EG_ERR_UNSUPPORTED, "eg_stem_conv: C=%d", c);
    hipLaunchKernelGGL(stem_conv_kernel, dim3(batch * h), dim3(256), 3 * (wdt + 2) * sizeof(float), (hipStream_t)stream, x, w9xc, bias, scale, shift, y,
                       batch, h, wdt, c);
    return eg_check_launch("stem_conv");
}

extern "C" int eg_se_gate(const float* gap_partial, int32_t tiles, const float* w1, const float* b1, const float* w2,
                          const float* b2, float* gate, int32_t batch, int32_t c, int32_t hw, void* stream) {
    EG_REQUIRE(gap_partial && w1 && b1 && w2 && b2 && gate && batch > 0, EG_ERR_BAD_ARG, "eg_se_gate: null pointer");
    EG_REQUIRE(c % 8 == 0 && c <= 256 && (c <= 128 ? 128 % c : 256 % c) == 0, EG_ERR_UNSUPPORTED, "eg_se_gate: C=%d", c);
    hipLaunchKernelGGL(se_gate_kernel, dim3(batch), dim3(c <= 128 ? 128 : 256), 0, (hipStream_t)stream, gap_partial, tiles, w1, b1, w2, b2,
                       gate, c, 1.0f / (float)hw);
    return eg_check_launch("se_gate");
}

namespace {
int se_gate_pre_launch(const float* t1, const float* gap_partial, int32_t tiles, const float* conv2_w, const float* scale2,
                       const float* shift2, const float* w1, const float* b1, const float* w2, const float* b2, float* gate,
                       int32_t batch, int32_t h, int32_t wdt, int32_t c, void* stream, const float* ds_scale, const float* ds_shift, float* sc_vec) {
    EG_REQUIRE(t1 && gap_partial && conv2_w && scale2 && shift2 && w1 && b1 && w2 && b2 && gate && batch > 0 && h > 1 && wdt > 1, EG_ERR_BAD_ARG,
               "eg_se_gate_pre: null pointer or empty shape");
    EG_REQUIRE(c % 8 == 0 && c <= 256 && 256 % c == 0 && eg_aligned16(conv2_w), EG_ERR_UNSUPPORTED, "eg_se_gate_pre: C=%d", c);
    const size_t smem = sizeof(float) * (5 * GP_T + 9 * (size_t)c + GP_T + c + (c >> 3) + 4);
    EG_REQUIRE(!sc_vec || (ds_scale && ds_shift), EG_ERR_BAD_ARG, "eg_se_gate_pre: the shortcut vectors need the downsample BatchNorm");
    hipLaunchKernelGGL(se_gate_pre_kernel, dim3(batch), dim3(GP_T), smem, (hipStream_t)stream, t1, gap_partial, tiles, conv2_w, scale2, shift2, w1,
                       b1, w2, b2, gate, h, wdt, c, ds_scale, ds_shift, sc_vec);
    return eg_check_launch("se_gate_pre");
}
}

extern "C" int eg_se_gate_pre(const float* t1, const float* gap_partial, int32_t tiles, const float* conv2_w, const float* scale2,
                              const float* shift2, const float* w1, const float* b1, const float* w2, const float* b2, float* gate,
                              int32_t batch, int32_t h, int32_t wdt, int32_t c, void* stream) {
    return se_gate_pre_launch(t1, gap_partial, tiles, conv2_w, scale2, shift2, w1, b1, w2, b2, gate, batch, h, wdt, c, stream, nullptr, nullptr, nullptr);
}

extern "C" int eg_se_block_fused(const float* x, const float* conv1_w, const float* scale1, const float* shift1, const float* conv2_w, const float* scale2,
                                 const float* shift2, const float* se_w1, const float* se_b1, const float* se_w2, const float* se_b2, const float* ds_w,
                                 const float* ds_scale, const float* ds_shift, float* t1, float* out, float* gap_partial, float* gate, float* sc_vec,
                                 int32_t batch, int32_t h, int32_t wdt, int32_t cin, int32_t cout, int32_t stride, int32_t precision, void* stream) {
    EG_REQUIRE(x && conv1_w && scale1 && shift1 && conv2_w && scale2 && shift2 && t1 && out && gap_partial && gate, EG_ERR_BAD_ARG, "eg_se_block_fused: null pointer");
    EG_REQUIRE(ds_w ? (ds_scale && ds_shift && sc_vec) : (cin == cout && stride == 1), EG_ERR_BAD_ARG,
               "eg_se_block_fused: a downsample needs its BatchNorm and the shortcut vectors; an identity shortcut needs cin == cout and stride 1");
    EG_REQUIRE(stride == 1 || stride == 2, EG_ERR_UNSUPPORTED, "eg_se_block_fused: stride %d", stride);
    const int ho = (h + 2 - 3) / stride + 1, wo = (wdt + 2 - 3) / stride + 1;
    if (int rc = eg_conv3x3(x, conv1_w, nullptr, scale1, shift1, t1, gap_partial, batch, h, wdt, cin, cout, stride, 1, 0, precision, stream)) return rc;
    const int tiles1 = eg_conv3x3_gap_tiles(h, wdt, cin, cout, stride);
    if (int rc = se_gate_pre_launch(t1, gap_partial, tiles1, conv2_w, scale2, shift2, se_w1, se_b1, se_w2, se_b2, gate, batch, ho, wo, cout, stream,
                                    ds_w ? ds_scale : nullptr, ds_w ? ds_shift : nullptr, ds_w ? sc_vec : nullptr)) return rc;
    if (!ds_w) return eg_conv3x3_se(t1, conv2_w, nullptr, scale2, shift2, gate, x, out, nullptr, batch, ho, wo, cout, cout, 1, 0, 0, precision, stream);
    const ShortcutArgs sc{x, ds_w, sc_vec, h, wdt, cin, stride};
    return conv3x3_dispatch(t1, conv2_w, nullptr, nullptr, nullptr, nullptr, nullptr, out, nullptr, nullptr, batch, ho, wo, cout, cout, 1, 0, 0, precision, stream,
                            nullptr, nullptr, nullptr, &sc);
}

extern "C" int eg_se_residual_relu(const float* y, const float* gate, const float* x_in, const float* ds_w,
                                   const float* ds_scale, const float* ds_shift, float* out, int32_t batch, int32_t ho,
                                   int32_t wo, int32_t c, int32_t h_in, int32_t w_in, int32_t cin, int32_t stride, void* stream) {
    EG_REQUIRE(y && gate && x_in && out && batch > 0, EG_ERR_BAD_ARG, "eg_se_residual_relu: null pointer");
    hipStream_t st = (hipStream_t)stream;
    if (!ds_w) {
        EG_REQUIRE(cin == c && h_in == ho && w_in == wo, EG_ERR_BAD_ARG, "eg_se_residual_relu: identity shortcut shape mismatch");
        const size_t n4 = (size_t)batch * ho * wo * c / 4;
        const int blocks = (int)((n4 + 255) / 256 < 8192 ? (n4 + 255) / 256 : 8192);
        hipLaunchKernelGGL(se_tail_identity_kernel, dim3(blocks), dim3(256), 0, st, reinterpret_cast<const f4*>(y), gate,
                           reinterpret_cast<const f4*>(x_in), reinterpret_cast<f4*>(out), n4, ho * wo * (c / 4), c / 4);
        return eg_check_launch("se_tail");
    }
    EG_REQUIRE(ds_scale && ds_shift, EG_ERR_BAD_ARG, "eg_se_residual_relu: downsample BN missing");
    const size_t total = (size_t)batch * ho * wo * (c / 4);
    const int blocks = (int)((total + 255) / 256 < 4096 ? (total + 255) / 256 : 4096);
    if (cin == 32 && c == 64)
        hipLaunchKernelGGL((se_tail_downsample_kernel<32, 64>), dim3(blocks), dim3(256), 32 * 64 * 4, st, y, gate, x_in, ds_w, ds_scale,
                           ds_shift, out, batch, ho, wo, h_in, w_in, stride);
    else if (cin == 64 && c == 128)
        hipLaunchKernelGGL((se_tail_downsample_kernel<64, 128>), dim3(blocks), dim3(256), 64 * 128 * 4, st, y, gate, x_in, ds_w, ds_scale,
                           ds_shift, out, batch, ho, wo, h_in, w_in, stride);
    else if (cin == 128 && c == 256) {
        if (int rc = eg_ensure_dynamic_lds(reinterpret_cast<const void*>(se_tail_downsample_kernel<128, 256>), 128 * 256 * 4, "eg_se_residual_relu")) return rc;
        hipLaunchKernelGGL((se_tail_downsample_kernel<128, 256>), dim3(blocks < 1024 ? blocks : 1024), dim3(256), 128 * 256 * 4, st, y, gate,
                           x_in, ds_w, ds_scale, ds_shift, out, batch, ho, wo, h_in, w_in, stride);
    } else {
        eg_set_error("eg_se_residual_relu: unsupported downsample %d->%d", cin, c);
        return EG_ERR_UNSUPPORTED;
    }
    return eg_check_launch("se_tail_downsample");
}
```

### emotiongestures_amd/csrc/generator.hip

```cpp
#include "common.h"
#include <string>
#include <vector>
#include <algorithm>
#include <string.h>
#include <map>
#include <mutex>

static thread_local char g_err[512] = "";
void eg_set_error(const char* fmt, ...) {
    va_list ap;
    va_start(ap, fmt);
    vsnprintf(g_err, sizeof(g_err), fmt, ap);
    va_end(ap);
}
extern "C" const char* eg_last_error(void) { return g_err; }
std::atomic<long long> g_eg_launches{0};
extern "C" int64_t eg_launch_count(void) { return (int64_t)g_eg_launches.load(std::memory_order_relaxed); }
bool g_eg_launch_hist = [] { const char* e = getenv("EG_LAUNCH_HIST"); return e && e[0] == '1'; }();
namespace {
std::mutex g_hist_mu;
std::map<std::string, long long> g_hist;
}
void egi_count_launch(const char* what) {
    std::lock_guard<std::mutex> lk(g_hist_mu);
// ... 179 lines not shown
}
void add_bn(Layout& L, const std::string& prefix, int n, int npad, int64_t& scale, int64_t& shift) {
    scale = L.add(prefix, EG_PACK_BN_SCALE, n, npad, 0, 0, npad);
    shift = L.add(prefix, EG_PACK_BN_SHIFT, n, npad, 0, 0, npad);
}
LinW add_linear_cat(Layout& L, const std::vector<std::string>& prefixes, int n_each, int k, bool bias) {
    LinW w;
    const int n = n_each * (int)prefixes.size();
    w.n = n; w.k = k; w.npad = (int)eg_round_up(n, 64); w.kpad = (int)eg_round_up(k, 64);
    std::string wk, bk;
    for (size_t i = 0; i < prefixes.size(); ++i) {
        wk += (i ? "|" : "") + prefixes[i] + ".weight";
        bk += (i ? "|" : "") + prefixes[i] + ".bias";
    }
    w.w = L.add(wk, EG_PACK_LINEAR, n, k, w.npad, w.kpad, (int64_t)w.npad * w.kpad * 2);
    if (bias) w.b = L.vec(bk, n, w.npad);
    return w;
}
LinW add_linear_fold(Layout& L, const std::string& chains, int n, int k, int kpad_force = 0, int npad_force = 0) {
    LinW w;
    w.n = n; w.k = k;
    w.npad = npad_force ? npad_force : (int)eg_round_up(n, 64);
    w.kpad = kpad_force ? kpad_force : (int)eg_round_up(k, 64);
    w.w = L.add(chains, EG_PACK_LINEAR_FOLD, n, k, w.npad, w.kpad, (int64_t)w.npad * w.kpad * 2);
    w.b = L.add(chains, EG_PACK_BIAS_FOLD, n, w.npad, 0, 0, w.npad);
    return w;
}
MhaW add_mha(Layout& L, const std::string& p, int d, bool self_attn) {
    MhaW m;
    if (self_attn) {
        m.qkv = add_linear_cat(L, {p + ".w_qs", p + ".w_ks", p + ".w_vs"}, d, d, false);
    } else {
        m.q = add_linear(L, p + ".w_qs", d, d, false);
        m.kv = add_linear_cat(L, {p + ".w_ks", p + ".w_vs"}, d, d, false);
    }
    m.o = add_linear(L, p + ".fc", d, d, false);
    m.ln_g = L.raw(p + ".layer_norm.weight", d);
    m.ln_b = L.raw(p + ".layer_norm.bias", d);
    return m;
}
FfnW add_ffn(Layout& L, const std::string& p, int d, int di) {
    FfnW f;
    f.w1 = add_linear(L, p + ".w_1", di, d, true);
    f.w2 = add_linear(L, p + ".w_2", d, di, true);
    f.ln_g = L.raw(p + ".layer_norm.weight", d);
    f.ln_b = L.raw(p + ".layer_norm.bias", d);
    return f;
}

struct Carver {
    int64_t off = 0;
    int64_t take(int64_t floats) {
        const int64_t o = off;
        off = eg_round_up(off + floats * (int64_t)sizeof(float), 256);
        return o;
    }
};

}

struct EgGenerator {
    EgGeneratorConfig cfg;
    Layout L;
    int H1, W1, H2, W2, H3, W3, HW3, Dpad, stages[3] = {3, 4, 6}, filters[3] = {32, 64, 128};
    int64_t stem_w, stem_b, stem_scale, stem_shift;
    std::vector<BlockW> blocks;
    ConvW final_conv;
    LinW a_fc1, a_fc2, emosem0, emo2, sem2, fus0, fus2, cls[4], post[4], prior_h0, prior_h2, txt_dec;
    bool fuse_se = true;
    bool fold = false;
    bool shared_chip = false;
    LinW f_audio, f_emo, f_sem, f_post, f_prior;
    int64_t pos_table;
    std::vector<MhaW> enc_attn, dec_attn;
    std::vector<FfnW> enc_ffn, dec_ffn;
    int64_t pc_w1, pc_b1, pc_s1, pc_t1, pc_w2, pc_b2, pc_s2, pc_t2;
    int64_t sp_w0, sp_b0, sp_w1, sp_b1, tc_w0, tc_b0, tc_w1, tc_b1, tm_w0, tm_b0, tm_w1, tm_b1;
    int64_t emb;
    struct TcnConv { LinW tap0, tap1, taps; int64_t bias; };
    std::vector<TcnConv> tcn;
    int64_t txt_fc1_w, txt_fc1_b;
    int Cpad;
    bool keep_taps = false;
    bool concurrent = false;
    mutable hipStream_t side[2] = {nullptr, nullptr};
    mutable hipEvent_t ev_fork = nullptr, ev_join[2] = {nullptr, nullptr};
    int ensure_streams() const {
        if (side[0]) return EG_OK;
        for (int i = 0; i < 2; ++i) {
            if (hipStreamCreateWithFlags(&side[i], hipStreamNonBlocking) != hipSuccess ||
                hipEventCreateWithFlags(&ev_join[i], hipEventDisableTiming) != hipSuccess) {
                eg_set_error("cannot create side stream/event");
                return EG_ERR_HIP;
            }
        }
        if (hipEventCreateWithFlags(&ev_fork, hipEventDisableTiming) != hipSuccess) { eg_set_error("cannot create event"); return EG_ERR_HIP; }
        return EG_OK;
    }
    ~EgGenerator() {
        for (int i = 0; i < 2; ++i) {
            if (side[i]) (void)hipStreamDestroy(side[i]);
            if (ev_join[i]) (void)hipEventDestroy(ev_join[i]);
        }
        if (ev_fork) (void)hipEventDestroy(ev_fork);
    }
};

namespace {

struct GenWs {
    int64_t act[3], gap, gate, scv, amap, afc1, afeat, emo_t, emo, sem_t, sem, cls_part, cls_h[3], cls_out;
    int64_t fus_in, fus_h, fusion, xa, xb, q, qkv, ao, proj, ffn_h, im_x[2], im_enc, im_h, im_a[3], im_p[2];
    int64_t prior_cat, prior_h, prior_enc, prior_rep, tm_mem, tm_pe, tm_gram, post_a, post_b, post_c, pose;
    int64_t t_emb, t_a, t_b, t_c, t_out, im_t[3], t_zero;
    int64_t tap_stem, tap_l[3];
    int64_t total;
};

GenWs carve(const EgGenerator* g, int B, int NB = 0) {
    if (NB <= 0) NB = B;
    const EgGeneratorConfig& c = g->cfg;
    GenWs w;
    Carver cv;
    const int64_t BF = (int64_t)B * c.frames, D = c.d_model, NF = (int64_t)NB * c.frames;
    const int64_t act = (int64_t)B * g->H1 * g->W1 * 32;
    for (int i = 0; i < 3; ++i) w.act[i] = cv.take(act);
    {
        int64_t gap_per_clip = 0;
        int h = g->H1, wd = g->W1;
        for (const BlockW& b : g->blocks) {
            const int ho = (h + 2 - 3) / b.stride + 1, wo = (wd + 2 - 3) / b.stride + 1;
            const int64_t need = (int64_t)eg_conv3x3_gap_tiles(ho, wo, b.cout, b.cout, 1) * b.cout;
            gap_per_clip = need > gap_per_clip ? need : gap_per_clip;
            const int64_t need1 = (int64_t)eg_conv3x3_gap_tiles(h, wd, b.cin, b.cout, b.stride) * b.cout;
            gap_per_clip = need1 > gap_per_clip ? need1 : gap_per_clip;
            h = ho; wd = wo;
        }
        w.gap = cv.take((int64_t)B * gap_per_clip);
    }
    w.gate = cv.take((int64_t)B * 128);
    w.scv = cv.take((int64_t)3 * B * 128);
    w.amap = cv.take(BF * g->HW3);
    w.afc1 = cv.take(BF * D); w.afeat = cv.take(BF * D);
    w.emo_t = cv.take(BF * D * 2); w.emo = cv.take(BF * D); w.sem_t = cv.take(16); w.sem = cv.take(BF * D);
    w.cls_part = cv.take((int64_t)(c.frames > 64 ? c.frames : 64) * B * D);
    w.cls_h[0] = cv.take((int64_t)B * D); w.cls_h[1] = cv.take((int64_t)B * 256); w.cls_h[2] = cv.take((int64_t)B * 64);
    w.cls_out = cv.take((int64_t)B * 16);
    w.fus_in = cv.take(NF * D); w.fus_h = cv.take(NF * D); w.fusion = cv.take(NF * D);
    w.xa = cv.take(NF * D); w.xb = cv.take(NF * D);
    w.q = cv.take(NF * D); w.qkv = cv.take(NF * D * 3); w.ao = cv.take(NF * D); w.proj = cv.take(NF * D);
    w.ffn_h = cv.take(NF * c.d_inner);
    {
        const int64_t N64 = eg_round_up(NF, 64), B64 = eg_round_up(BF, 64), KX = D > g->Dpad ? D : g->Dpad;
        w.im_x[0] = cv.take(N64 * KX); w.im_x[1] = cv.take(N64 * KX); w.im_enc = cv.take(N64 * D); w.im_h = cv.take(N64 * c.d_inner);
        w.im_a[0] = cv.take(B64 * D); w.im_a[1] = cv.take(B64 * D); w.im_a[2] = cv.take(B64 * D * 2);
        w.im_p[0] = cv.take(B64 * D); w.im_p[1] = cv.take(B64 * D);
    }
    w.prior_cat = cv.take(BF * g->Dpad); w.prior_h = cv.take(BF * D); w.prior_enc = cv.take(BF * D);
    w.prior_rep = cv.take(NB > B ? NF * D : 16);
    w.tm_mem = cv.take((int64_t)B * c.pose_dim); w.tm_pe = cv.take((int64_t)B * c.chunk + 16); w.tm_gram = cv.take((int64_t)c.pose_dim * c.chunk);
    w.post_a = cv.take(NF * D * 4); w.post_b = cv.take(NF * D); w.post_c = cv.take(NF * g->Dpad); w.pose = cv.take(NF * c.pose_dim);
    const int64_t BT = (int64_t)B * c.text_len;
    w.t_emb = cv.take(BT * g->Cpad); w.t_a = cv.take(BT * g->Cpad); w.t_b = cv.take(BT * g->Cpad); w.t_c = cv.take(BT * g->Cpad);
    w.t_out = cv.take(BT * 512);
    for (int i = 0; i < 3; ++i) w.im_t[i] = cv.take(eg_round_up(BT, 64) * g->Cpad);
    w.t_zero = cv.take((int64_t)g->Cpad * 32);
// ... 10 lines not shown

inline float* P(void* ws, int64_t off) { return reinterpret_cast<float*>(reinterpret_cast<char*>(ws) + off); }

int run_linear(const float* arena, const LinW& w, const float* x, int lda, float* y, int ldc, int m, int relu, const float* res1,
               int ldr, int prec, hipStream_t st, int n_override = 0) {
    return eg_linear(x, lda, arena + w.w, w.kpad, w.b >= 0 ? arena + w.b : nullptr, res1, nullptr, ldr, y, ldc, m,
                     n_override ? n_override : w.n, w.kpad <= lda ? w.kpad : w.k, relu, 0, 0, prec, st);
}

int run_conv(const float* arena, const ConvW& c, const float* x, float* y, float* gap, int B, int h, int w, int relu, int nchw,
             int prec, hipStream_t st) {
    return eg_conv3x3(x, arena + c.w, c.bias >= 0 ? arena + c.bias : nullptr, c.scale >= 0 ? arena + c.scale : nullptr,
                      c.shift >= 0 ? arena + c.shift : nullptr, y, gap, B, h, w, c.cin, c.cout, c.stride, relu, nchw, prec, st);
}

struct Act { float* f = nullptr; int ld = 0; void* img = nullptr; int kimg = 0; };
inline Act act(float* f, int ld, void* img = nullptr, int kimg = 0) { Act a; a.f = f; a.ld = ld; a.img = img; a.kimg = kimg; return a; }

int lin(const EgGenerator* g, const float* arena, const LinW& w, const Act& x, int xk0, const Act& y, bool want_f32, int m, int relu,
        const float* res1, int ldr, hipStream_t st, int n_override = 0, int splits = 0, float* partial = nullptr) {
    const bool img_ok = g->cfg.precision != EG_PREC_F32;
    EgiLinear p;
    p.w = arena + w.w; p.ldw = w.kpad; p.bias = w.b >= 0 ? arena + w.b : nullptr;
    p.res1 = res1; p.ldr = ldr; p.m = m; p.n = n_override ? n_override : w.n; p.relu = relu; p.precision = g->cfg.precision;
    p.shared_chip = g->shared_chip ? 1 : 0;
    if (img_ok && x.img) {
        p.ximg = x.img; p.xK = x.kimg; p.xk0 = xk0; p.k = w.kpad;
    } else {
        p.x = x.f + xk0; p.lda = x.ld; p.k = (w.kpad <= x.ld - xk0 || w.kpad <= x.ld) && (x.ld >= w.kpad) ? w.kpad : w.k;
    }
    const bool yimg = img_ok && y.img;
    if (yimg) { p.yimg = y.img; p.yK = y.kimg; }
    if (want_f32 || !yimg) { p.y = y.f; p.ldc = y.ld; }
    if (splits > 1 && img_ok && x.img && !yimg) { p.splits = splits; p.partial = partial; }
    return egi_linear(p, st);
}

int run_mha(const EgGenerator* g, const float* arena, const MhaW& m, const Act& xq, const Act& xkv, const Act& out, const GenWs& w,
            void* ws, int B, int Lq, int Lk, hipStream_t st) {
    const int D = g->cfg.d_model;
    float *qkv = P(ws, w.qkv), *ao = P(ws, w.ao), *pr = P(ws, w.proj);
    void* aimg = g->cfg.precision != EG_PREC_F32 ? P(ws, w.im_h) : nullptr;
    if (!xkv.f) {
        EG_TRY(lin(g, arena, m.qkv, xq, 0, act(qkv, 3 * D), true, B * Lq, 0, nullptr, 0, st));
        EG_TRY(egi_attention(qkv, 3 * D, qkv + D, 3 * D, qkv + 2 * D, 3 * D, ao, D, nullptr, aimg, B, g->cfg.n_head, Lq, Lk, g->cfg.d_k, g->cfg.precision, st));
    } else {
        float* q = P(ws, w.q);
        EG_TRY(lin(g, arena, m.q, xq, 0, act(q, D), true, B * Lq, 0, nullptr, 0, st));
        EG_TRY(lin(g, arena, m.kv, xkv, 0, act(qkv, 2 * D), true, B * Lk, 0, nullptr, 0, st));
        EG_TRY(egi_attention(q, D, qkv, 2 * D, qkv + D, 2 * D, ao, D, nullptr, aimg, B, g->cfg.n_head, Lq, Lk, g->cfg.d_k, g->cfg.precision, st));
    }
    EG_TRY(lin(g, arena, m.o, act(ao, D, aimg, D), 0, act(pr, D), true, B * Lq, 0, xq.f, D, st));
    return egi_layernorm(pr, arena + m.ln_g, arena + m.ln_b, out.f, g->cfg.precision != EG_PREC_F32 ? out.img : nullptr, B * Lq, D, 1e-6f, st);
}

int run_mha_kv(const EgGenerator* g, const float* arena, const MhaW& m, const Act& xq, const float* kv, const Act& out, const GenWs& w,
               void* ws, int B, int Lq, int Lk, hipStream_t st) {
    const int D = g->cfg.d_model;
    float *q = P(ws, w.q), *ao = P(ws, w.ao), *pr = P(ws, w.proj);
    void* aimg = g->cfg.precision != EG_PREC_F32 ? P(ws, w.im_h) : nullptr;
    EG_TRY(lin(g, arena, m.q, xq, 0, act(q, D), true, B * Lq, 0, nullptr, 0, st));
    EG_TRY(egi_attention(q, D, kv, 2 * D, kv + D, 2 * D, ao, D, nullptr, aimg, B, g->cfg.n_head, Lq, Lk, g->cfg.d_k, g->cfg.precision, st));
    EG_TRY(lin(g, arena, m.o, act(ao, D, aimg, D), 0, act(pr, D), true, B * Lq, 0, xq.f, D, st));
    return egi_layernorm(pr, arena + m.ln_g, arena + m.ln_b, out.f, g->cfg.precision != EG_PREC_F32 ? out.img : nullptr, B * Lq, D, 1e-6f, st);
}

int run_ffn(const EgGenerator* g, const float* arena, const FfnW& f, const Act& x, const Act& out, const GenWs& w, void* ws, int rows,
            hipStream_t st) {
    const int D = g->cfg.d_model, DI = g->cfg.d_inner;
    float *h = P(ws, w.ffn_h), *pr = P(ws, w.proj);
    const Act hid = act(h, DI, P(ws, w.im_h), DI);
    EG_TRY(lin(g, arena, f.w1, x, 0, hid, false, rows, 1, nullptr, 0, st));
    const int sp = (g->cfg.precision != EG_PREC_F32 && rows <= 64 && DI >= 2048 && 4 * D <= DI) ? 4 : 0;
    EG_TRY(lin(g, arena, f.w2, hid, 0, act(pr, D), true, rows, 0, x.f, D, st, 0, sp, h));
    return egi_layernorm(pr, arena + f.ln_g, arena + f.ln_b, out.f, g->cfg.precision != EG_PREC_F32 ? out.img : nullptr, rows, D, 1e-6f, st);
}


int run_audio_tower(const EgGenerator* g, const float* arena, const float* spec, const GenWs& w, void* ws, int B, hipStream_t st) {
    const int prec = g->cfg.precision, F = g->cfg.frames, D = g->cfg.d_model;
    float* bufs[3] = {P(ws, w.act[0]), P(ws, w.act[1]), P(ws, w.act[2])};
    float *gap = P(ws, w.gap), *gate = P(ws, w.gate);
    int xi = 0, h = g->H1, wd = g->W1, bi = 0;
    EG_TRY(eg_stem_conv(spec, arena + g->stem_w, arena + g->stem_b, arena + g->stem_scale, arena + g->stem_shift, bufs[0], B, g->H1,
                        g->W1, 32, st));
    if (g->keep_taps)
        EG_HIP_TRY(hipMemcpyAsync(P(ws, w.tap_stem), bufs[0], sizeof(float) * (size_t)B * g->H1 * g->W1 * 32, hipMemcpyDeviceToDevice, st), "tap copy");
    for (int s = 0; s < 3; ++s) {
        for (int j = 0; j < g->stages[s]; ++j, ++bi) {
            const BlockW& bw = g->blocks[bi];
            const int t1 = (xi + 1) % 3, t2 = (xi + 2) % 3;
            const int ho = (h + 2 - 3) / bw.stride + 1, wo = (wd + 2 - 3) / bw.stride + 1;
            if (g->fuse_se && (!bw.ds || prec != EG_PREC_F32)) {
                EG_TRY(eg_se_block_fused(bufs[xi], arena + bw.c1.w, arena + bw.c1.scale, arena + bw.c1.shift, arena + bw.c2.w, arena + bw.c2.scale,
                                         arena + bw.c2.shift, arena + bw.se_w1, arena + bw.se_b1, arena + bw.se_w2, arena + bw.se_b2,
                                         bw.ds ? arena + bw.ds_wb : nullptr, bw.ds ? arena + bw.ds_scale : nullptr, bw.ds ? arena + bw.ds_shift : nullptr,
                                         bufs[t1], bufs[t2], gap, gate, P(ws, w.scv), B, h, wd, bw.cin, bw.cout, bw.stride, prec, st));
                xi = t2; h = ho; wd = wo;
                continue;
            }
            EG_TRY(run_conv(arena, bw.c1, bufs[xi], bufs[t1], nullptr, B, h, wd, 1, 0, prec, st));
            EG_TRY(run_conv(arena, bw.c2, bufs[t1], bufs[t2], gap, B, ho, wo, 0, 0, prec, st));
            const int tiles = eg_conv3x3_gap_tiles(ho, wo, bw.cout, bw.cout, 1);
            EG_TRY(eg_se_gate(gap, tiles, arena + bw.se_w1, arena + bw.se_b1, arena + bw.se_w2, arena + bw.se_b2, gate, B, bw.cout,
                              ho * wo, st));
            EG_TRY(eg_se_residual_relu(bufs[t2], gate, bufs[xi], bw.ds ? arena + bw.ds_w : nullptr, bw.ds ? arena + bw.ds_scale : nullptr,
                                       bw.ds ? arena + bw.ds_shift : nullptr, bufs[t1], B, ho, wo, bw.cout, h, wd, bw.cin, bw.stride, st));
            xi = t1; h = ho; wd = wo;
        }
        if (g->keep_taps)
            EG_HIP_TRY(hipMemcpyAsync(P(ws, w.tap_l[s]), bufs[xi], sizeof(float) * (size_t)B * h * wd * g->filters[s], hipMemcpyDeviceToDevice, st), "tap copy");
    }
    float* amap = P(ws, w.amap);
    EG_TRY(run_conv(arena, g->final_conv, bufs[xi], amap, nullptr, B, h, wd, 0, 1, prec, st));
    if (g->fold) return lin(g, arena, g->f_audio, act(amap, g->HW3), 0, act(P(ws, w.afeat), D, P(ws, w.im_a[1]), D), true, B * F, 0, nullptr, 0, st);
    const Act h1 = act(P(ws, w.afc1), D, P(ws, w.im_a[0]), D);
    EG_TRY(lin(g, arena, g->a_fc1, act(amap, g->HW3), 0, h1, false, B * F, 0, nullptr, 0, st));
    return lin(g, arena, g->a_fc2, h1, 0, act(P(ws, w.afeat), D, P(ws, w.im_a[1]), D), true, B * F, 0, nullptr, 0, st);
}

int causal_conv(const EgGenerator* g, const float* arena, const EgGenerator::TcnConv& cv, void* ximg, const void* zero, float* y, void* yimg,
                const float* res2, int rows, int d, int L, hipStream_t st) {
    EgiLinear p;
    p.ximg = ximg; p.xK = g->Cpad; p.w = arena + cv.taps.w; p.ldw = cv.taps.kpad; p.bias = arena + cv.bias; p.res2 = res2; p.ldr = g->Cpad;
    p.y = y; p.ldc = g->Cpad; p.yimg = yimg; p.yK = g->Cpad; p.m = rows; p.n = g->Cpad; p.k = cv.taps.kpad; p.relu = 1;
    p.precision = g->cfg.precision; p.shared_chip = g->shared_chip ? 1 : 0;
    p.xs_shift = d; p.xs_period = L; p.xzero = zero;
    return egi_linear(p, st);
}

bool text_one_launch(const EgGenerator* g) {
    if (g->cfg.precision == EG_PREC_F32 || g->cfg.embed_dim != g->cfg.tcn_hidden || g->Cpad != (int)eg_round_up(g->cfg.tcn_hidden, 64)) return false;
    const char* e = getenv("EG_TEXT_TAPS");
    return !(e && e[0] == '2');
}

int run_text(const EgGenerator* g, const float* arena, const int64_t* text, float* out, const GenWs& w, void* ws, int B, hipStream_t st) {
    const EgGeneratorConfig& c = g->cfg;
    const int L = c.text_len, C = c.tcn_hidden, ld = g->Cpad, rows = B * L, prec = c.precision;
    float *x = P(ws, w.t_emb), *h1 = P(ws, w.t_a), *h2 = P(ws, w.t_b), *y = P(ws, w.t_c);
    if (text_one_launch(g)) {
        void *xi = P(ws, w.im_t[0]), *hi = P(ws, w.im_t[1]), *yi = P(ws, w.im_t[2]), *zero = P(ws, w.t_zero);
        EG_TRY(egi_embedding_img(text, arena + g->emb, x, xi, zero, rows, c.embed_dim, ld, c.n_words, st));
        for (int i = 0; i < c.tcn_layers; ++i) {
            const bool last = i + 1 == c.tcn_layers;
            EG_TRY(causal_conv(g, arena, g->tcn[2 * i], xi, zero, nullptr, hi, nullptr, rows, 1 << i, L, st));
            EG_TRY(causal_conv(g, arena, g->tcn[2 * i + 1], hi, zero, y, last ? nullptr : yi, x, rows, 1 << i, L, st));
            float* t = x; x = y; y = t;
            void* ti = xi; xi = yi; yi = ti;
        }
        EG_TRY(egi_time_linear(x, arena + g->txt_fc1_w, arena + g->txt_fc1_b, h1, B, L, C, ld, st));
        return eg_linear(h1, ld, arena + g->txt_dec.w, g->txt_dec.kpad, arena + g->txt_dec.b, nullptr, nullptr, 0, out, 512, rows, 512, C, 0,
                         0, 0, prec, st);
    }
    EG_TRY(egi_embedding(text, arena + g->emb, x, rows, c.embed_dim, ld, c.n_words, st));
    for (int i = 0; i < c.tcn_layers; ++i) {
        const int d = 1 << i;
        const EgGenerator::TcnConv& c1 = g->tcn[2 * i];
        const EgGenerator::TcnConv& c2 = g->tcn[2 * i + 1];
        EG_TRY(eg_linear(x, ld, arena + c1.tap0.w, c1.tap0.kpad, arena + c1.bias, nullptr, nullptr, 0, h1, ld, rows, C, C, 0, d, L, prec, st));
        EG_TRY(eg_linear(x, ld, arena + c1.tap1.w, c1.tap1.kpad, nullptr, h1, nullptr, ld, h1, ld, rows, C, C, 1, 0, 0, prec, st));
        EG_TRY(eg_linear(h1, ld, arena + c2.tap0.w, c2.tap0.kpad, arena + c2.bias, nullptr, nullptr, 0, h2, ld, rows, C, C, 0, d, L, prec, st));
        EG_TRY(eg_linear(h1, ld, arena + c2.tap1.w, c2.tap1.kpad, nullptr, h2, x, ld, y, ld, rows, C, C, 1, 0, 0, prec, st));
        float* t = x; x = y; y = t;
    }
    EG_TRY(egi_time_linear(x, arena + g->txt_fc1_w, arena + g->txt_fc1_b, h1, B, L, C, ld, st));
    return eg_linear(h1, ld, arena + g->txt_dec.w, g->txt_dec.kpad, arena + g->txt_dec.b, nullptr, nullptr, 0, out, 512, rows, 512, C, 0,
                     0, 0, prec, st);
}

int run_prior(const EgGenerator* g, const float* arena, const float* prior, const GenWs& w, void* ws, int B, hipStream_t st) {
    const EgGeneratorConfig& c = g->cfg;
    EgiPriorW pw;
    memset(&pw, 0, sizeof(pw));
    pw.w1 = arena + g->pc_w1; pw.b1 = arena + g->pc_b1; pw.s1 = arena + g->pc_s1; pw.t1 = arena + g->pc_t1;
// ... 59 lines not shown
    return lin(g, arena, g->post[3], pc, 0, act(pose, c.pose_dim), true, rows, 0, nullptr, 0, st);
}

int run_decoder(const EgGenerator* g, const float* arena, const Act& prior_enc, const Act& enc_out, float* const* kv, float* pose,
                const GenWs& w, void* ws, int NB, hipStream_t st) {
    const EgGeneratorConfig& c = g->cfg;
    const int F = c.frames, D = c.d_model, rows = NB * F;
    void *im0 = P(ws, w.im_x[0]), *im1 = P(ws, w.im_x[1]);
    float *xb = P(ws, w.xb), *da = P(ws, w.fus_h);
    Act dx = prior_enc;
    for (int l = 0; l < c.n_layers; ++l) {
        const Act mid = act(xb, D, im0, D);
        const Act nxt = act(da, D, im1, D);
        if (kv) EG_TRY(run_mha_kv(g, arena, g->dec_attn[l], dx, kv[l], mid, w, ws, NB, F, F, st));
        else EG_TRY(run_mha(g, arena, g->dec_attn[l], dx, enc_out, mid, w, ws, NB, F, F, st));
        EG_TRY(run_ffn(g, arena, g->dec_ffn[l], mid, nxt, w, ws, rows, st));
        dx = nxt;
    }
    return run_post(g, arena, dx, pose, w, ws, rows, st);
}

int run_transformer(const EgGenerator* g, const float* arena, const Act& fusion_in, const Act& prior_enc, float* pose, const GenWs& w,
                    void* ws, int NB, hipStream_t st) {
    Act enc_out;
    EG_TRY(run_encoder(g, arena, fusion_in, enc_out, w, ws, NB, st));
    return run_decoder(g, arena, prior_enc, enc_out, nullptr, pose, w, ws, NB, st);
}

int run_heads(const EgGenerator* g, const float* arena, float* emo, float* sem, float* pred, const GenWs& w, void* ws, int B, hipStream_t st) {
    const EgGeneratorConfig& c = g->cfg;
    const int F = c.frames, D = c.d_model, rows = B * F, prec = c.precision;
    const Act afeat = act(P(ws, w.afeat), D, P(ws, w.im_a[1]), D), es = act(P(ws, w.emo_t), 2 * D, P(ws, w.im_a[2]), 2 * D);
    if (g->fold) {
        EG_TRY(lin(g, arena, g->f_emo, afeat, 0, act(emo, D), true, rows, 0, nullptr, 0, st));
        EG_TRY(lin(g, arena, g->f_sem, afeat, 0, act(sem, D), true, rows, 0, nullptr, 0, st));
    } else {
        EG_TRY(lin(g, arena, g->emosem0, afeat, 0, es, false, rows, 0, nullptr, 0, st));
        EG_TRY(lin(g, arena, g->emo2, es, 0, act(emo, D), true, rows, 0, nullptr, 0, st));
        EG_TRY(lin(g, arena, g->sem2, es, D, act(sem, D), true, rows, 0, nullptr, 0, st));
    }
    const int K0 = F * D;
    EG_TRY(eg_linear_splitk(emo, K0, arena + g->cls[0].w, g->cls[0].kpad, arena + g->cls[0].b, P(ws, w.cls_h[0]), D, B, D, K0, 1,
                            F, P(ws, w.cls_part), prec, st));
    EG_TRY(run_linear(arena, g->cls[1], P(ws, w.cls_h[0]), D, P(ws, w.cls_h[1]), 256, B, 1, nullptr, 0, prec, st));
    EG_TRY(run_linear(arena, g->cls[2], P(ws, w.cls_h[1]), 256, P(ws, w.cls_h[2]), 64, B, 1, nullptr, 0, prec, st));
    return run_linear(arena, g->cls[3], P(ws, w.cls_h[2]), 64, pred, 8, B, 0, nullptr, 0, prec, st);
}

int validate_cfg(const EgGeneratorConfig& c) {
    EG_REQUIRE(c.frames > c.prior_frames && c.prior_frames >= c.chunk && c.chunk > 0, EG_ERR_BAD_ARG, "config: frames/prior/chunk inconsistent");
    EG_REQUIRE(c.d_model % 64 == 0 && c.d_model >= 64 && c.d_model <= 2048, EG_ERR_UNSUPPORTED, "config: d_model=%d", c.d_model);
    EG_REQUIRE(c.d_k == 64 && c.n_head * c.d_k == c.d_model, EG_ERR_UNSUPPORTED, "config: heads*d_k must equal d_model with d_k=64");
    EG_REQUIRE(c.n_mels % 16 == 0 && c.n_mels <= 512 && c.spec_len >= 4, EG_ERR_UNSUPPORTED, "config: spectrogram %dx%d", c.n_mels, c.spec_len);
    EG_REQUIRE(c.frames <= 128, EG_ERR_UNSUPPORTED, "config: frames=%d > 128 (final conv width)", c.frames);
    EG_REQUIRE(c.embed_dim == c.tcn_hidden && c.embed_dim % 4 == 0, EG_ERR_UNSUPPORTED, "config: TCN needs embed_dim == hidden, %%4");
    EG_REQUIRE(c.variant == 0 || c.variant == 1, EG_ERR_BAD_ARG, "config: variant=%d", c.variant);
    EG_REQUIRE(c.precision >= 0 && c.precision <= 2, EG_ERR_BAD_ARG, "config: precision=%d", c.precision);
    EG_REQUIRE(c.n_position >= c.frames, EG_ERR_BAD_ARG, "config: n_position < frames");
    EG_REQUIRE(c.pose_dim > 0 && c.pose_dim <= 1024 && c.n_words > 0 && c.text_len > 0 && c.text_len <= 128, EG_ERR_BAD_ARG, "config: sizes");
    return EG_OK;
}

}

extern "C" int eg_generator_default_config(EgGeneratorConfig* c) {
    EG_REQUIRE(c, EG_ERR_BAD_ARG, "null config");
    memset(c, 0, sizeof(*c));
    c->frames = 34; c->pose_dim = 126; c->prior_frames = 4; c->chunk = 4; c->d_model = 512; c->d_inner = 2048; c->n_layers = 3;
    c->n_head = 8; c->d_k = 64; c->n_mels = 128; c->spec_len = 124; c->text_len = 60; c->n_words = 200; c->embed_dim = 300;
    c->tcn_hidden = 300; c->tcn_layers = 3; c->variant = 0; c->precision = g_default_precision; c->n_position = 60;
    return EG_OK;
}

extern "C" int eg_generator_create(const EgGeneratorConfig* cfg, EgGenerator** out) {
    EG_REQUIRE(cfg && out, EG_ERR_BAD_ARG, "eg_generator_create: null pointer");
    EG_TRY(validate_cfg(*cfg));
    EgGenerator* g = new EgGenerator();
    g->cfg = *cfg;
    g->keep_taps = cfg->reserved[0] != 0;
    g->concurrent = cfg->reserved[1] != 0;
    g->fold = cfg->reserved[2] != 0;
    g->fuse_se = cfg->reserved[3] == 0;
    g->shared_chip = cfg->reserved[4] != 0;
    const EgGeneratorConfig& c = g->cfg;
    g->H1 = c.n_mels; g->W1 = c.spec_len;
    g->H2 = (g->H1 - 1) / 2 + 1; g->W2 = (g->W1 - 1) / 2 + 1;
    g->H3 = (g->H2 - 1) / 2 + 1; g->W3 = (g->W2 - 1) / 2 + 1;
    g->HW3 = g->H3 * g->W3;
    if (g->HW3 % 8 != 0) { delete g; eg_set_error("config: final map %dx%d not a multiple of 8", g->H3, g->W3); return EG_ERR_UNSUPPORTED; }
    g->Dpad = (int)eg_round_up(c.pose_dim, 64);
    g->Cpad = (int)eg_round_up(c.tcn_hidden, 64);
    Layout& L = g->L;
    const int D = c.d_model, F = c.frames, P_ = c.prior_frames, PL = F - P_, PD = c.pose_dim;
    const std::string fe = "audio_encoder.feat_extractor";
    g->stem_w = L.add(fe + ".conv1.weight", EG_PACK_STEM, 32, 0, 0, 0, 9 * 32);
    g->stem_b = L.raw(fe + ".conv1.bias", 32);
    add_bn(L, fe + ".bn1", 32, 32, g->stem_scale, g->stem_shift);
    int inpl = 32;
    for (int s = 0; s < 3; ++s) {
        const int planes = g->filters[s];
        for (int j = 0; j < g->stages[s]; ++j) {
            BlockW b;
            const std::string p = fe + ".layer" + std::to_string(s + 1) + "." + std::to_string(j);
            b.stride = (s > 0 && j == 0) ? 2 : 1;
            b.cin = inpl; b.cout = planes;
            b.c1 = add_conv3(L, p + ".conv1", inpl, planes, b.stride);
            add_bn(L, p + ".bn1", planes, planes, b.c1.scale, b.c1.shift);
            b.c2 = add_conv3(L, p + ".conv2", planes, planes, 1);
            add_bn(L, p + ".bn2", planes, planes, b.c2.scale, b.c2.shift);
            b.se_w1 = L.raw(p + ".se.fc.0.weight", planes / 8 * planes);
            b.se_b1 = L.raw(p + ".se.fc.0.bias", planes / 8);
            b.se_w2 = L.raw(p + ".se.fc.2.weight", planes * (planes / 8));
            b.se_b2 = L.raw(p + ".se.fc.2.bias", planes);
            b.ds = (b.stride != 1 || inpl != planes);
            if (b.ds) {
                b.ds_w = L.add(p + ".downsample.0.weight", EG_PACK_CONV1X1, planes, inpl, 0, 0, (int64_t)inpl * planes);
                b.ds_wb = L.add(p + ".downsample.0.weight", EG_PACK_CONV1X1_BF16, planes, inpl, 0, 0, (int64_t)inpl * planes);
                add_bn(L, p + ".downsample.1", planes, planes, b.ds_scale, b.ds_shift);
            }
            g->blocks.push_back(b);
            inpl = planes;
        }
    }
    g->final_conv = add_conv3(L, "audio_encoder.final_conv1", 128, F, 1);
    if (g->final_conv.coutp > 64) {
        g->final_conv.coutp = 128;
        L.entries.back().dims[2] = 128;
        L.total -= L.entries.back().numel;
        L.entries.back().numel = (int64_t)9 * 128 * 128 * 2;
        L.total += L.entries.back().numel;
    }
    g->final_conv.bias = L.vec("audio_encoder.final_conv1.bias", F, g->final_conv.coutp);
    add_bn(L, "audio_encoder.bn1", F, g->final_conv.coutp, g->final_conv.scale, g->final_conv.shift);
    if (g->fold) {
        g->f_audio = add_linear_fold(L, "audio_encoder.fc2@audio_encoder.fc1", D, g->HW3);
        g->f_emo = add_linear_fold(L, "emotion_proj.2@emotion_proj.0", D, D);
        g->f_sem = add_linear_fold(L, "semantic_proj.2@semantic_proj.0", D, D);
    } else {
        g->a_fc1 = add_linear(L, "audio_encoder.fc1", D, g->HW3, true);
        g->a_fc2 = add_linear(L, "audio_encoder.fc2", D, D, true);
        g->emosem0 = add_linear_cat(L, {"emotion_proj.0", "semantic_proj.0"}, D, D, true);
        g->emo2 = add_linear(L, "emotion_proj.2", D, D, true);
        g->sem2 = add_linear(L, "semantic_proj.2", D, D, true);
    }
    g->fus0 = add_linear(L, "fusion_proj.0", D, D, true); g->fus2 = add_linear(L, "fusion_proj.2", D, D, true);
    g->cls[0] = add_linear(L, "emotion_classifer_header.0", D, F * D, true);
    g->cls[1] = add_linear(L, "emotion_classifer_header.2", 256, D, true);
    g->cls[2] = add_linear(L, "emotion_classifer_header.4", 64, 256, true);
    g->cls[3] = add_linear(L, "emotion_classifer_header.6", 8, 64, true);
    const std::string pp = "prior_seq_encoder";
    if (g->fold) {
        g->f_post = add_linear_fold(L, "post_projector.6@post_projector.4@post_projector.2@post_projector.0", PD, D);
        g->f_prior = add_linear_fold(L, pp + ".post_header.2@" + pp + ".post_header.0", D, PD, g->Dpad, 0);
    } else {
        g->post[0] = add_linear(L, "post_projector.0", D * 4, D, true);
        g->post[1] = add_linear(L, "post_projector.2", D, D * 4, true);
        g->post[2] = add_linear(L, "post_projector.4", PD, D, true, 0, g->Dpad);
        g->post[3] = add_linear(L, "post_projector.6", PD, PD, true, g->Dpad, 0);
        g->prior_h0 = add_linear(L, pp + ".post_header.0", D, PD, true, g->Dpad, 0);
        g->prior_h2 = add_linear(L, pp + ".post_header.2", D, D, true);
    }
    g->pc_w1 = L.raw(pp + ".pred_conv.0.weight", (int64_t)PL * P_ * 3); g->pc_b1 = L.raw(pp + ".pred_conv.0.bias", PL);
    add_bn(L, pp + ".pred_conv.2", PL, PL, g->pc_s1, g->pc_t1);
    g->pc_w2 = L.raw(pp + ".pred_conv.3.weight", (int64_t)PL * PL * 3); g->pc_b2 = L.raw(pp + ".pred_conv.3.bias", PL);
    add_bn(L, pp + ".pred_conv.5", PL, PL, g->pc_s2, g->pc_t2);
    if (c.variant == 1) {
// ... 675 lines not shown
```

### emotiongestures_amd/ops.py

```python
from __future__ import annotations

import ctypes as C
from typing import Optional

import numpy as np
import torch

from . import _lib as L
from . import packing
from ._host import need_cuda as _need_cuda, ptr as _ptr, stream as _stream


def _dev(t):
    return t.device


def pack_linear_weight(w: torch.Tensor, device) -> torch.Tensor:
    n, k = w.shape
    npad, kpad = (n + 63) // 64 * 64, (k + 63) // 64 * 64
    if w.is_cuda and w.device == torch.device(device) and w.dtype == torch.float32:
        lib = L.load()
        wd = w.detach().contiguous()
        img = torch.empty(int(lib.eg_linear_packed_floats(n, k)), dtype=torch.float32, device=wd.device)
        L.check(lib.eg_pack_linear_device(_ptr(wd), k, n, k, 0, _ptr(img), _stream(wd.device)), "eg_pack_linear_device")
# ... 7 lines not shown
        lib = L.load()
        wd = w.detach().contiguous()
        img = torch.empty(int(lib.eg_conv3x3_packed_floats(wd.shape[1], opad)), dtype=torch.float32, device=wd.device)
        L.check(lib.eg_pack_conv3x3_device(_ptr(wd), wd.shape[0], wd.shape[1], 0, _ptr(img), _stream(wd.device)), "eg_pack_conv3x3_device")
        return img, opad
    return torch.from_numpy(packing._pack_conv3x3(w.detach().cpu().float(), opad)).to(device), opad


def _padvec(v: Optional[torch.Tensor], npad: int, device, fill=0.0):
    if v is None:
        return None
    out = torch.full((npad,), fill, dtype=torch.float32, device=device)
    out[: v.numel()] = v.detach().to(device, torch.float32).reshape(-1)
    return out


def conv3x3(x_nhwc, weight_oihw, bias=None, scale=None, shift=None, stride=1, relu=False, nchw_out=False, want_gap=False,
            precision="f32", packed=None):
    lib = L.load()
    x = _need_cuda(x_nhwc, "x")
    dev = x.device
    B, H, W, Cin = x.shape
    Cout = weight_oihw.shape[0]
    if packed is not None:
        wp, bias_p, scale_p, shift_p = packed
    else:
        wp, bias_p, scale_p, shift_p = conv3x3_pack(weight_oihw, bias, scale, shift, dev)
    Ho, Wo = (H - 1) // stride + 1, (W - 1) // stride + 1
    y = torch.empty((B, Cout, Ho * Wo) if nchw_out else (B, Ho, Wo, Cout), device=dev)
    gap = None
    tiles = lib.eg_conv3x3_gap_tiles(H, W, Cin, Cout, stride)
    if want_gap:
        gap = torch.empty(B, tiles, Cout, device=dev)
    L.check(lib.eg_conv3x3(_ptr(x), _ptr(wp), _ptr(bias_p), _ptr(scale_p), _ptr(shift_p), _ptr(y), _ptr(gap), B, H, W, Cin, Cout,
                           stride, int(relu), int(nchw_out), L.precision_code(precision), _stream(dev)), "eg_conv3x3")
    return (y, gap) if want_gap else y


def conv3x3_pack(weight_oihw, bias, scale, shift, device):
    wp, opad = pack_conv3x3_weight(weight_oihw, device)
    return wp, _padvec(bias, opad, device), _padvec(scale, opad, device), _padvec(shift, opad, device)


def stem_conv(x, weight, bias, scale, shift):
    lib = L.load()
    x = _need_cuda(x, "x")
    dev = x.device
    B, H, W = x.shape
    Cc = weight.shape[0]
    w9 = weight.detach().reshape(Cc, 9).t().contiguous().to(dev, torch.float32)
    y = torch.empty(B, H, W, Cc, device=dev)
    L.check(lib.eg_stem_conv(_ptr(x), _ptr(w9), _ptr(_need_cuda(bias, "bias")), _ptr(_need_cuda(scale, "scale")),
                             _ptr(_need_cuda(shift, "shift")), _ptr(y), B, H, W, Cc, _stream(dev)), "eg_stem_conv")
    return y


def se_gate(gap_partial, w1, b1, w2, b2, hw: int):
    lib = L.load()
    g = _need_cuda(gap_partial, "gap")
    dev = g.device
    B, tiles, Cc = g.shape
    gate = torch.empty(B, Cc, device=dev)
    L.check(lib.eg_se_gate(_ptr(g), tiles, _ptr(_need_cuda(w1, "w1")), _ptr(_need_cuda(b1, "b1")), _ptr(_need_cuda(w2, "w2")),
                           _ptr(_need_cuda(b2, "b2")), _ptr(gate), B, Cc, hw, _stream(dev)), "eg_se_gate")
    return gate


def se_residual_relu(y, gate, x_in, ds_weight=None, ds_scale=None, ds_shift=None, stride=1):
    lib = L.load()
    y, gate, x_in = _need_cuda(y, "y"), _need_cuda(gate, "gate"), _need_cuda(x_in, "x_in")
    dev = y.device
    B, Ho, Wo, Cc = y.shape
    _, Hi, Wi, Cin = x_in.shape
    dsw = None
    if ds_weight is not None:
        dsw = ds_weight.detach().reshape(Cc, Cin).t().contiguous().to(dev, torch.float32)
        ds_scale, ds_shift = _need_cuda(ds_scale, "ds_scale"), _need_cuda(ds_shift, "ds_shift")
    out = torch.empty_like(y)
    L.check(lib.eg_se_residual_relu(_ptr(y), _ptr(gate), _ptr(x_in), _ptr(dsw), _ptr(ds_scale), _ptr(ds_shift), _ptr(out), B, Ho, Wo,
                                    Cc, Hi, Wi, Cin, stride, _stream(dev)), "eg_se_residual_relu")
    return out


def se_block_fused(x_nhwc, c1, c2, se_w1, se_b1, se_w2, se_b2, cout, stride=1, ds_weight=None, ds_scale=None, ds_shift=None, precision="bf16x3"):
    lib = L.load()
    x = _need_cuda(x_nhwc, "x")
    dev = x.device
    B, H, W, Cin = x.shape
    Ho, Wo = (H - 1) // stride + 1, (W - 1) // stride + 1
    tiles = lib.eg_conv3x3_gap_tiles(H, W, Cin, cout, stride)
    t1, out = torch.empty(B, Ho, Wo, cout, device=dev), torch.empty(B, Ho, Wo, cout, device=dev)
    gap, gate = torch.empty(B, tiles, cout, device=dev), torch.empty(B, cout, device=dev)
    dsw = scv = None
    if ds_weight is not None:
        dsw = torch.from_numpy(packing._pack_conv1x1_bf16(ds_weight.detach().cpu().float())).to(dev)
        scv = torch.empty(3, B, cout, device=dev)
        ds_scale, ds_shift = _need_cuda(ds_scale, "ds_scale"), _need_cuda(ds_shift, "ds_shift")
    L.check(lib.eg_se_block_fused(_ptr(x), _ptr(c1[0]), _ptr(c1[2]), _ptr(c1[3]), _ptr(c2[0]), _ptr(c2[2]), _ptr(c2[3]), _ptr(_need_cuda(se_w1, "w1")),
                                  _ptr(_need_cuda(se_b1, "b1")), _ptr(_need_cuda(se_w2, "w2")), _ptr(_need_cuda(se_b2, "b2")), _ptr(dsw), _ptr(ds_scale),
                                  _ptr(ds_shift), _ptr(t1), _ptr(out), _ptr(gap), _ptr(gate), _ptr(scv), B, H, W, Cin, cout, stride,
                                  L.precision_code(precision), _stream(dev)), "eg_se_block_fused")
    return out


def linear(x, weight, bias=None, res1=None, res2=None, relu=False, a_shift=0, a_seq=0, precision="f32", packed=None):
    lib = L.load()
    x = _need_cuda(x, "x")
    dev = x.device
    M, K = x.shape
    N = weight.shape[0]
    wp, npad, kpad = packed if packed is not None else pack_linear_weight(weight, dev)
    bias_p = _padvec(bias, npad, dev)
    y = torch.empty(M, N, device=dev)
    r1 = _need_cuda(res1, "res1") if res1 is not None else None
    r2 = _need_cuda(res2, "res2") if res2 is not None else None
    L.check(lib.eg_linear(_ptr(x), K, _ptr(wp), kpad, _ptr(bias_p), _ptr(r1), _ptr(r2), N, _ptr(y), N, M, N, K, int(relu), a_shift,
                          a_seq, L.precision_code(precision), _stream(dev)), "eg_linear")
    return y


def linear_splitk(x, weight, bias=None, relu=False, splits=8, precision="f32", packed=None):
    lib = L.load()
    x = _need_cuda(x, "x")
    dev = x.device
    M, K = x.shape
    N = weight.shape[0]
    wp, npad, kpad = packed if packed is not None else pack_linear_weight(weight, dev)
    bias_p = _padvec(bias, npad, dev)
    y = torch.empty(M, N, device=dev)
    part = torch.empty(splits + 1, M, N, device=dev)
    L.check(lib.eg_linear_splitk(_ptr(x), K, _ptr(wp), kpad, _ptr(bias_p), _ptr(y), N, M, N, K, int(relu), splits, _ptr(part),
                                 L.precision_code(precision), _stream(dev)), "eg_linear_splitk")
    return y


def layernorm(x, gamma, beta, eps=1e-6):
    lib = L.load()
    x = _need_cuda(x, "x")
    dev = x.device
    rows, d = x.reshape(-1, x.shape[-1]).shape
    y = torch.empty_like(x)
    L.check(lib.eg_layernorm(_ptr(x), _ptr(_need_cuda(gamma, "gamma")), _ptr(_need_cuda(beta, "beta")), _ptr(y), rows, d, eps,
                             _stream(dev)), "eg_layernorm")
    return y


def _attention_mask_bytes(mask, B, Lq, Lk, dev):
    m = mask
    if m.dim() == 4:
        if m.shape[1] != 1:
            raise NotImplementedError("attention mask: per-head masks are not used by the reference (the head axis is broadcast)")
        m = m[:, 0]
    if m.dim() == 2:
        m = m[:, None, :]
    rows = Lq if m.shape[1] != 1 else 1
    m = (m != 0).expand(B, rows, Lk).to(device=dev, dtype=torch.uint8).contiguous()
    return m, rows * Lk, (Lk if rows > 1 else 0)


def attention(q, k, v, heads: int, want_attn=False, precision="f32", mask=None):
    lib = L.load()
    q, k, v = _need_cuda(q, "q"), _need_cuda(k, "k"), _need_cuda(v, "v")
    dev = q.device
    B, Lq, D = q.shape
    Lk = k.shape[1]
    out = torch.empty_like(q)
    attn = torch.empty(B, heads, Lq, Lk, device=dev) if want_attn else None
    if mask is not None:
        mb, sb, sq = _attention_mask_bytes(mask, B, Lq, Lk, dev)
        L.check(lib.eg_attention_masked(_ptr(q), D, _ptr(k), D, _ptr(v), D, _ptr(mb), sb, sq, _ptr(out), D, _ptr(attn), B, heads, Lq, Lk,
                                        D // heads, L.precision_code(precision), _stream(dev)), "eg_attention_masked")
        return (out, attn) if want_attn else out
    L.check(lib.eg_attention(_ptr(q), D, _ptr(k), D, _ptr(v), D, _ptr(out), D, _ptr(attn), B, heads, Lq, Lk, D // heads,
                             L.precision_code(precision), _stream(dev)), "eg_attention")
    return (out, attn) if want_attn else out


def multi_head_attention(xq, xkv, wq, wk, wv, wo, ln_g, ln_b, heads: int, precision="f32", want_attn=True, packed=None):
    lib = L.load()
    xq, xkv = _need_cuda(xq, "q"), _need_cuda(xkv, "kv")
    dev = xq.device
    B, Lq, D = xq.shape
    Lk = xkv.shape[1]
    packs = packed if packed is not None else [pack_linear_weight(w, dev)[0] for w in (wq, wk, wv, wo)]
    nbytes = lib.eg_mha_workspace_bytes(B, Lq, Lk, D, heads)
# ... 98 lines not shown
```

### include/emogest.h

```cpp
#ifndef EMOGEST_H
#define EMOGEST_H

#include <stddef.h>
#include <stdint.h>

#ifdef __cplusplus
extern "C" {
#endif

typedef enum EgStatus {
    EG_OK = 0,
    EG_ERR_BAD_ARG = -1,
    EG_ERR_UNSUPPORTED = -2,
    EG_ERR_WORKSPACE = -3,
    EG_ERR_HIP = -4,
    EG_ERR_ALIGN = -5
} EgStatus;

typedef enum EgPrecision {
    EG_PREC_F32 = 0,
    EG_PREC_BF16X3 = 1,
    EG_PREC_BF16 = 2
} EgPrecision;

// ... 221 lines not shown
#define EG_UNWRAP_TILE_FRAMES 64
int eg_articulate_euler(const float* track, int32_t rows, int32_t T, int32_t joints, const int32_t* orders, const void* d_orders,
                        const int32_t* d_frames, int32_t draws, int32_t frame_unit, const float* d_mean, int32_t basis, int32_t degrees,
                        int32_t L, int32_t M, float* euler, int64_t out_stride, void* stream);
int eg_articulate_rot6d_euler(const float* euler, int32_t rows, int32_t T, int32_t joints, const int32_t* orders, const void* d_orders,
                              const int32_t* d_frames, int32_t draws, int32_t frame_unit, const float* d_mean, int32_t basis,
                              int32_t degrees, float* rot6d, void* stream);
int64_t eg_angle_unwrap_workspace_bytes(int32_t rows, int32_t T, int32_t C);
int eg_angle_unwrap(float* angles, int32_t rows, int32_t T, int32_t C, const int32_t* d_frames, int32_t draws, int32_t frame_unit,
                    double period, void* workspace, int64_t workspace_bytes, void* stream);

#define EG_SMOOTH_MAX_WINDOW 31
#define EG_SMOOTH_TILE_FRAMES 64
#define EG_SMOOTH_TILE_COLS 64
int eg_smooth_design(int32_t K, int32_t p, int32_t d, double delta, double* table64, float* table32);
int32_t eg_smooth_tile_frames(void);
int32_t eg_smooth_tile_cols(void);
int eg_smooth_tracks(const float* track, int32_t rows, int32_t T, int32_t D, int32_t K, const float* d_table, const int32_t* frames,
                     const int32_t* d_frames, int32_t draws, int32_t frame_unit, float* out, void* stream);
int64_t eg_smooth_stream_state_bytes(int32_t rows, int32_t D, int32_t K);
int eg_smooth_stream_reset(void* state, int32_t rows, int32_t D, int32_t K, const int32_t* row_mask, void* stream);
int eg_smooth_stream_push(void* state, int32_t rows, int32_t H, int32_t D, int32_t K, const float* d_table, const float* chunk,
                          const int32_t* d_valid, float* out, void* stream);
int eg_smooth_stream_tail(const void* state, int32_t rows, int32_t P, int32_t D, int32_t K, const float* d_table, const float* tail_rows,
                          float* out, void* stream);

#define EG_BEAT_MAX_FRAMES 1024
int eg_beat_tables(float* h_melfb_t , float* h_window , float* h_twiddle ,
                   int32_t* h_band );
int64_t eg_beat_workspace_bytes(int32_t batch, int32_t n_samples);
int eg_beat_align(const float* audio, int32_t batch, int32_t n_samples, const float* pose, int32_t frames, int32_t pose_dim,
                  int32_t pose_fps, int32_t t_start, int32_t t_end, double sigma, int32_t order, const float* d_melfb_t,
                  const float* d_window, const float* d_twiddle, const int32_t* d_band, void* workspace, int64_t workspace_bytes,
                  double* score, int32_t* n_audio_beats, float* oenv, float* rms, uint8_t* audio_beats, uint8_t* pose_beats,
                  void* stream);

int64_t eg_beat_tracks_meta_ints(int32_t recordings);
int eg_beat_tracks_meta(const int32_t* lengths, const int32_t* frames , const int32_t* t_end ,
                        int32_t pose_fps, int32_t recordings, int32_t* meta);
int64_t eg_beat_tracks_workspace_bytes(const int32_t* lengths, const int32_t* frames , int32_t recordings, int32_t draws,
                                       int32_t Tmax);
int eg_beat_align_tracks(const float* audio, int32_t recordings, int64_t stride, const int32_t* lengths, const int32_t* d_meta,
                         const float* pose, int32_t draws, int32_t Tmax, int32_t pose_dim, const int32_t* frames, int32_t pose_fps,
                         int32_t t_start, const int32_t* t_end, double sigma, int32_t order, const float* d_melfb_t, const float* d_window,
                         const float* d_twiddle, const int32_t* d_band, void* workspace, int64_t workspace_bytes, double* score,
                         int32_t* n_audio_beats, float* oenv, float* rms, uint8_t* audio_beats, uint8_t* pose_beats, void* stream);
int eg_beat_tracks_scan(const uint8_t* d_cand, const int32_t* lengths, int32_t recordings, const int32_t* d_meta, void* workspace,
                        int64_t workspace_bytes, int32_t* events, int32_t* counts, void* stream);

#define EG_TAKE_CHUNK_FRAMES 16
#define EG_TAKE_MAX_DRAWS 64
int64_t eg_take_meta_ints(int32_t recordings);
int eg_take_meta(const int32_t* frames, int32_t recordings, int32_t* meta);
int eg_track_rows_pack(const float* track, int32_t recordings, int32_t draws, int32_t Tmax, int32_t pose_dim, const int32_t* frames,
                       const int32_t* d_meta, float* rows, void* stream);
int64_t eg_take_distance_workspace_bytes(const int32_t* frames, int32_t recordings, int32_t draws);
int eg_take_distance(const float* feat, int32_t recordings, int32_t draws, int32_t feat_dim, const int32_t* frames, const int32_t* d_meta,
                     int32_t span , void* workspace, int64_t workspace_bytes, double* distance, double* diversity,
                     void* stream);


int eg_conv3x3(const float* x, const float* w, const float* bias, const float* scale, const float* shift,
               float* y, float* gap_partial, int32_t batch, int32_t h, int32_t wdt, int32_t cin, int32_t cout,
               int32_t stride, int32_t relu, int32_t nchw_out, int32_t precision, void* stream);
int32_t eg_conv3x3_gap_tiles(int32_t h, int32_t wdt, int32_t cin, int32_t cout, int32_t stride);
int32_t eg_conv3x3_channel_split(int32_t batch, int32_t h, int32_t wdt, int32_t cin, int32_t cout, int32_t stride, int32_t precision);
int eg_conv3x3_se(const float* x, const float* w_packed, const float* bias, const float* scale, const float* shift, const float* gate,
                  const float* residual, float* y, float* gap_partial, int32_t batch, int32_t h, int32_t wdt, int32_t cin, int32_t cout,
                  int32_t stride, int32_t relu, int32_t nchw_out, int32_t precision, void* stream);
int eg_conv3x3_res_masked(const float* x, const float* w_packed, const float* residual, const uint32_t* res_bits, float* y, int32_t batch, int32_t h,
                          int32_t wdt, int32_t cin, int32_t cout, int32_t precision, void* stream);
int eg_conv3x3_sq(const float* x, const float* w_packed, const float* bias, float* y, float* gap_partial, float* gap_sq_partial, int32_t batch,
                  int32_t h, int32_t wdt, int32_t cin, int32_t cout, int32_t stride, int32_t relu, int32_t precision, void* stream);
int eg_conv3x3_sq_in_affine(const float* x, const float* in_scale, const float* in_shift, const float* w_packed, const float* bias, float* y,
                            float* gap_partial, float* gap_sq_partial, int32_t batch, int32_t h, int32_t wdt, int32_t cin, int32_t cout, int32_t stride,
                            int32_t relu, int32_t precision, void* stream);
int eg_se_gate_pre(const float* t1, const float* gap_partial, int32_t tiles, const float* conv2_w_packed, const float* scale2,
                   const float* shift2, const float* w1, const float* b1, const float* w2, const float* b2, float* gate,
                   int32_t batch, int32_t h, int32_t wdt, int32_t c, void* stream);
int eg_se_block_fused(const float* x, const float* conv1_w, const float* scale1, const float* shift1, const float* conv2_w, const float* scale2,
                      const float* shift2, const float* se_w1, const float* se_b1, const float* se_w2, const float* se_b2, const float* ds_w,
                      const float* ds_scale, const float* ds_shift, float* t1, float* out, float* gap_partial, float* gate, float* sc_vec,
                      int32_t batch, int32_t h, int32_t wdt, int32_t cin, int32_t cout, int32_t stride, int32_t precision, void* stream);
int64_t eg_conv3x3_packed_floats(int32_t cin, int32_t cout_pad);

int eg_stem_conv(const float* x, const float* w9xc, const float* bias, const float* scale, const float* shift,
                 float* y, int32_t batch, int32_t h, int32_t wdt, int32_t c, void* stream);

int eg_se_gate(const float* gap_partial, int32_t tiles, const float* w1, const float* b1, const float* w2,
               const float* b2, float* gate, int32_t batch, int32_t c, int32_t hw, void* stream);

int eg_se_residual_relu(const float* y, const float* gate, const float* x_in, const float* ds_w,
                        const float* ds_scale, const float* ds_shift, float* out, int32_t batch, int32_t ho,
                        int32_t wo, int32_t c, int32_t h_in, int32_t w_in, int32_t cin, int32_t stride, void* stream);

int eg_linear(const float* x, int32_t lda, const float* w, int32_t ldw, const float* bias,
              const float* res1, const float* res2, int32_t ldr, float* y, int32_t ldc,
              int32_t m, int32_t n, int32_t k, int32_t relu, int32_t a_shift, int32_t a_seq,
              int32_t precision, void* stream);
int eg_split_tiles(const float* x, int32_t lda, int32_t m, int32_t k, void* images, void* stream);
int eg_linear_presplit(const void* x_images, int32_t k_x, const float* w, int32_t ldw, const float* bias,
                       const float* res1, const float* res2, int32_t ldr, float* y, int32_t ldc,
                       int32_t m, int32_t n, int32_t k, int32_t relu, int32_t precision, void* stream);
int eg_linear_presplit_causal(const void* x_images, int32_t k_x, const void* zero_line, const float* w, int32_t ldw, const float* bias,
                              const float* res2, int32_t ldr, float* y, int32_t ldc, void* y_images, int32_t y_k, int32_t m, int32_t n,
                              int32_t k_tap, int32_t relu, int32_t shift, int32_t period, int32_t precision, void* stream);

int eg_linear_splitk(const float* x, int32_t lda, const float* w, int32_t ldw, const float* bias, float* y,
                     int32_t ldc, int32_t m, int32_t n, int32_t k, int32_t relu, int32_t splits,
                     float* partial, int32_t precision, void* stream);

typedef struct EgLinearArgs {
    const float* x; const float* w; const float* bias; const float* res1; const float* res2; float* y;
    const float* gate_src;
    const int32_t* drop_epoch;
    float* partial;
    const void* x_images;
    void* y_images;
    uint64_t drop_offset;
    int32_t lda, ldw, ldr, ldc, ldg;
    int32_t m, n, k, relu, precision, splits;
    int32_t k_x, y_k;
    uint32_t drop_seed;
    float drop_p;
} EgLinearArgs;
int eg_linear_ex(const EgLinearArgs* args, void* stream);

int eg_layernorm(const float* x, const float* gamma, const float* beta, float* y, int32_t rows, int32_t d,
                 float eps, void* stream);
int eg_layernorm_img(const float* x, const float* gamma, const float* beta, float* y, void* y_images, int32_t rows, int32_t d, float eps,
                     void* stream);

int eg_attention(const float* q, int32_t ldq, const float* k, int32_t ldk, const float* v, int32_t ldv,
                 float* out, int32_t ldo, float* attn, int32_t batch, int32_t heads, int32_t lq, int32_t lk,
                 int32_t dk, int32_t precision, void* stream);
int eg_attention_masked(const float* q, int32_t ldq, const float* k, int32_t ldk, const float* v, int32_t ldv, const uint8_t* mask,
                        int64_t mask_batch_stride, int32_t mask_query_stride, float* out, int32_t ldo, float* attn, int32_t batch,
                        int32_t heads, int32_t lq, int32_t lk, int32_t dk, int32_t precision, void* stream);

int64_t eg_mha_workspace_bytes(int32_t batch, int32_t lq, int32_t lk, int32_t d_model, int32_t heads);
int eg_multi_head_attention(const float* xq, const float* xkv, const float* wq, const float* wk, const float* wv,
                            const float* wo, const float* ln_g, const float* ln_b, float* out, float* attn,
                            int32_t batch, int32_t lq, int32_t lk, int32_t d_model, int32_t heads,
                            int32_t precision, void* workspace, int64_t workspace_bytes, void* stream);

int64_t eg_ffn_workspace_bytes(int32_t rows, int32_t d_model, int32_t d_inner);
int eg_positionwise_ffn(const float* x, const float* w1, const float* b1, const float* w2, const float* b2,
                        const float* ln_g, const float* ln_b, float* out, int32_t rows, int32_t d_model,
                        int32_t d_inner, int32_t precision, void* workspace, int64_t workspace_bytes, void* stream);

int eg_tcn_forward(const float* x, const float* w, float* y, int32_t batch, int32_t len, int32_t c,
                   int32_t levels, int32_t precision, void* workspace, int64_t workspace_bytes, void* stream);

int eg_add_rows_split(const float* a, const float* table, float* out, void* images, int64_t rows, int32_t d, int32_t period, void* stream);
int eg_add_rows(const float* a, const float* table, float* out, int64_t rows, int32_t d, int32_t period, void* stream);

int eg_time_linear(const float* x, const float* w, const float* bias, float* y, int32_t batch, int32_t len, int32_t c, int32_t ld, void* stream);

int eg_reparameterize(const float* mu, const float* logvar, const float* eps, float* z, int64_t n, void* stream);

int eg_conv1d(const float* x, const float* w, const float* bias, const float* scale, const float* shift, float* y, int32_t n,
              int32_t cin, int32_t cout, int32_t lin, int32_t k, int32_t stride, int32_t pad, int32_t act, void* stream);

int64_t eg_contrastive_workspace_bytes(int32_t n);
int eg_contrastive_loss(const float* face, const float* audio, int32_t n, int32_t d, float* cross, float* loss, float* acc,
                        void* workspace, int64_t workspace_bytes, void* stream);
// ... 118 lines not shown
```

Before: 26670 clips/s.

## Fuse stem conv into first SE block via in-pipeline and residual recompute

The stem 3x3 conv (1->32 channels, ReLU, affine) is no longer written to a 32-channel activation buffer. The first SE block's conv1 now recomputes it per tile from a spectrogram patch held in LDS, interleaving the stem FMAs with the MFMA taps. Conv2 recomputes the same stem output for its residual from a 3x3 spectrogram window. This removes the stem kernel launch and the write and two reads of a B*H*W*32 float tensor. In exchange it adds redundant VALU work, extra LDS, and scheduling barriers that could slow the MFMA loop.

```diff
diff --git a/emotiongestures_amd/_lib.py b/emotiongestures_amd/_lib.py
--- a/emotiongestures_amd/_lib.py
+++ b/emotiongestures_amd/_lib.py
@@ -158,6 +158,8 @@
     "eg_conv3x3_se": (C.c_int, [_P, _P, _P, _P, _P, _P, _P, _P, _P, _I, _I, _I, _I, _I, _I, _I, _I, _I, _P]),
     "eg_se_gate_pre": (C.c_int, [_P, _P, _I, _P, _P, _P, _P, _P, _P, _P, _P, _I, _I, _I, _I, _P]),
     "eg_se_block_fused": (C.c_int, [_P] * 19 + [_I] * 7 + [_P]),
+    "eg_se_block_fused_stem": (C.c_int, [_P] * 20 + [_I] * 4 + [_P]),
+    "eg_stem_fused_available": (_I, [_I]),
     "eg_conv3x3_gap_tiles": (_I, [_I, _I, _I, _I, _I]),
     "eg_conv3x3_channel_split": (_I, [_I, _I, _I, _I, _I, _I, _I]),
     "eg_stem_conv": (C.c_int, [_P, _P, _P, _P, _P, _P, _I, _I, _I, _I, _P]),
diff --git a/emotiongestures_amd/csrc/conv.hip b/emotiongestures_amd/csrc/conv.hip
--- a/emotiongestures_amd/csrc/conv.hip
+++ b/emotiongestures_amd/csrc/conv.hip
@@ -17,7 +17,24 @@
     unsigned int* dbg = nullptr;
     const float* sc_x = nullptr; const bf8* sc_whi = nullptr; const bf8* sc_wlo = nullptr; const float* sc_vec = nullptr;
     int sc_H = 0, sc_W = 0, sc_S = 2, sc_B = 0;
+    const float* st_x = nullptr; const float* st_w = nullptr; const float* st_b = nullptr; const float* st_scale = nullptr; const float* st_shift = nullptr;
 };
+__device__ __forceinline__ f4 stem_quad(const float (&x)[9], const f4 (&w)[9], const f4& bi, const f4& sc, const f4& sh) {
+    f4 v;
+#pragma unroll
+    for (int r = 0; r < 4; ++r) {
+        float acc = bi[r];
+#pragma unroll
+        for (int t = 0; t < 9; ++t) acc = fmaf(w[t][r], x[t], acc);
+        v[r] = fmaf(fmaxf(acc, 0.f), sc[r], sh[r]);
+    }
+    return v;
+}
+enum { STEM_NONE = 0, STEM_IN_PIPE = 1, STEM_RES = 2 };
+constexpr int STEM_PARAM_FLOATS = 9 * 32 + 3 * 32, STEM_PATCH_W = 36, STEM_PATCH_FLOATS = 8 * STEM_PATCH_W;
+__host__ __device__ constexpr size_t stem_lds_bytes(int stem) {
+    return stem == STEM_NONE ? 0 : sizeof(float) * (STEM_PARAM_FLOATS + (stem == STEM_IN_PIPE ? STEM_PATCH_FLOATS + 8 : 0));
+}
 __device__ __forceinline__ f4 residual_quad(const float* __restrict__ res, const unsigned* __restrict__ bits, size_t e) {
     f4 r = *reinterpret_cast<const f4*>(res + e);
     if (bits) {
@@ -577,13 +594,16 @@
     }
 }
 
-template <int TERMS, int TH = 4, bool STAMP = false>
+template <int TERMS, int TH = 4, bool STAMP = false, int STEM = STEM_NONE>
 __global__ __launch_bounds__(256, 2) void conv3x3_c32_persistent_kernel(ConvArgs a, const bf8* __restrict__ whi, const bf8* __restrict__ wlo,
                                                                      int total_tiles, int tiles_per_wg) {
     using G = ConvGeom<1, TH>;
     constexpr int CIN = 32, IW = G::IW, NPIX = G::NPIX, PL = G::PL, MT = TH / 2, NT = 2;
     constexpr int NIMG = (TERMS == 3) ? 2 : 1;
     constexpr int TILE = NIMG * 4 * PL, WTAP = 4 * 32, WIMG = 9 * WTAP;
+    constexpr bool STEM_PIPE = STEM == STEM_IN_PIPE;
+    static_assert(STEM == STEM_NONE || TH == 4, "the stem recompute lives behind the gap scratch of the 4-row variant");
+    static_assert(!STEM_PIPE || (G::IH + 2) * (IW + 2) <= STEM_PATCH_FLOATS, "the spectrogram patch of a tile's halo");
     static_assert(PL - NPIX >= 8 || TH == 4, "the gap scratch of the 8-row variant lives in the planes' padding slots");
     extern __shared__ __attribute__((aligned(16))) bf8 lds[];
     bf8* tile = lds;
@@ -591,6 +611,8 @@
     float* sred_base = reinterpret_cast<float*>(lds + TILE + NIMG * WIMG);
     const int sred_pitch = (TH == 4) ? 32 : PL * 4;
     float* sred = (TH == 4) ? sred_base : reinterpret_cast<float*>(tile + NPIX);
+    float* stp = sred_base + 2 * 4 * 32;
+    float* patch = stp + STEM_PARAM_FLOATS;
 
     const int tid = threadIdx.x, wave = tid >> 6, lane = tid & 63, li = lane & 15, kq = lane >> 4;
     const int wave_u = __builtin_amdgcn_readfirstlane(wave);
@@ -612,6 +634,10 @@
                                                  (__attribute__((address_space(3))) void*)(wl + img * WIMG + piece * 64), 16, 0, 0);
         }
     }
+    if constexpr (STEM != STEM_NONE) {
+        for (int i = tid; i < STEM_PARAM_FLOATS; i += 256)
+            stp[i] = i < 288 ? a.st_w[i] : i < 320 ? a.st_b[i - 288] : i < 352 ? a.st_scale[i - 320] : a.st_shift[i - 352];
+    }
 
     constexpr int NIT = (((NPIX + 7) / 8) * 32 + 255) / 256;
     int piy[NIT], pix[NIT], lslot[NIT];
@@ -625,7 +651,8 @@
     }
     const int oc8 = ((tid >> 3) & 3) * 8;
     f4 isc[2] = {(f4){1.f, 1.f, 1.f, 1.f}, (f4){1.f, 1.f, 1.f, 1.f}}, ish[2] = {(f4){0.f, 0.f, 0.f, 0.f}, (f4){0.f, 0.f, 0.f, 0.f}};
-    if (a.in_scale) {
+    const bool in_affine = STEM == STEM_NONE && a.in_scale;
+    if (in_affine) {
         isc[0] = *reinterpret_cast<const f4*>(a.in_scale + oc8); isc[1] = *reinterpret_cast<const f4*>(a.in_scale + oc8 + 4);
         ish[0] = *reinterpret_cast<const f4*>(a.in_shift + oc8); ish[1] = *reinterpret_cast<const f4*>(a.in_shift + oc8 + 4);
     }
@@ -640,9 +667,37 @@
         if (c.ty >= tiles_y) { c.ty -= tiles_y; ++c.b; }
         c.b += adv_b;
     };
+    auto window_load = [&](const float* __restrict__ sb, int cy, int cx, float (&x)[9]) {
+        unsigned ro[3], co[3];
+#pragma unroll
+        for (int k = 0; k < 3; ++k) {
+            ro[k] = (unsigned)(min(max(cy + k - 1, 0), a.H - 1) * a.W);
+            co[k] = (unsigned)min(max(cx + k - 1, 0), a.W - 1);
+        }
+#pragma unroll
+        for (int t = 0; t < 9; ++t) x[t] = sb[ro[t / 3] + co[t % 3]];
+    };
+    auto window_pad = [&](int cy, int cx, float (&x)[9]) {
+#pragma unroll
+        for (int t = 0; t < 9; ++t) {
+            const bool in = ((unsigned)(cy + t / 3 - 1) < (unsigned)a.H) & ((unsigned)(cx + t % 3 - 1) < (unsigned)a.W);
+            x[t] = in ? x[t] : 0.f;
+        }
+    };
+    float px[2] = {0.f, 0.f};
     auto load_tile = [&](const Coord& c) {
         const int b = c.b;
         const int iy0 = c.ty * TH - 1, ix0 = c.tx * 32 - 1;
+        if constexpr (STEM_PIPE) {
+            const float* __restrict__ sb = a.st_x + (size_t)b * a.H * a.W;
+#pragma unroll
+            for (int j = 0; j < 2; ++j) {
+                const int q = tid + j * 256, r = q / STEM_PATCH_W, cl = q - r * STEM_PATCH_W;
+                const int gy = iy0 - 1 + r, gx = ix0 - 1 + cl;
+                px[j] = sb[(unsigned)(min(max(gy, 0), a.H - 1) * a.W + min(max(gx, 0), a.W - 1))];
+            }
+            return;
+        }
         const float* __restrict__ xb = a.x + (size_t)b * a.H * a.W * CIN;
 #pragma unroll
         for (int it = 0; it < NIT; ++it) {
@@ -652,11 +707,62 @@
                 const float* src = xb + (gy * a.W + gx) * CIN + oc8;
                 pv[it][0] = *reinterpret_cast<const f4*>(src);
                 pv[it][1] = *reinterpret_cast<const f4*>(src + 4);
-                if (a.in_scale) {
+                if (in_affine) {
                     pv[it][0] = pv[it][0] * isc[0] + ish[0];
                     pv[it][1] = pv[it][1] * isc[1] + ish[1];
                 }
             }
+        }
+    };
+    auto stem_consts = [&](int ch, f4 (&wq)[9], f4& sbi, f4& ssc, f4& ssh) {
+#pragma unroll
+        for (int t = 0; t < 9; ++t) wq[t] = *reinterpret_cast<const f4*>(stp + t * 32 + ch);
+        sbi = *reinterpret_cast<const f4*>(stp + 288 + ch);
+        ssc = *reinterpret_cast<const f4*>(stp + 320 + ch);
+        ssh = *reinterpret_cast<const f4*>(stp + 352 + ch);
+    };
+    auto patch_write = [&](const Coord& c) {
+        const int iy0 = c.ty * TH - 1, ix0 = c.tx * 32 - 1;
+#pragma unroll
+        for (int j = 0; j < 2; ++j) {
+            const int q = tid + j * 256, r = q / STEM_PATCH_W, cl = q - r * STEM_PATCH_W;
+            const bool in = ((unsigned)(iy0 - 1 + r) < (unsigned)a.H) & ((unsigned)(ix0 - 1 + cl) < (unsigned)a.W);
+            if (q < STEM_PATCH_FLOATS) patch[q] = in ? px[j] : 0.f;
+        }
+    };
+    auto stem_begin = [&]() {
+        const f4 b0 = *reinterpret_cast<const f4*>(stp + 288 + oc8), b1 = *reinterpret_cast<const f4*>(stp + 288 + oc8 + 4);
+#pragma unroll
+        for (int it = 0; it < NIT; ++it) { pv[it][0] = b0; pv[it][1] = b1; }
+    };
+    auto stem_tap = [&](int t) {
+        const f4 w0 = *reinterpret_cast<const f4*>(stp + t * 32 + oc8), w1 = *reinterpret_cast<const f4*>(stp + t * 32 + oc8 + 4);
+#pragma unroll
+        for (int it = 0; it < NIT; ++it) {
+            const float x = patch[(piy[it] + t / 3) * STEM_PATCH_W + pix[it] + t % 3];
+#pragma unroll
+            for (int r = 0; r < 4; ++r) {
+                pv[it][0][r] = fmaf(w0[r], x, pv[it][0][r]);
+                pv[it][1][r] = fmaf(w1[r], x, pv[it][1][r]);
+            }
+            asm volatile("" : "+v"(pv[it][0]), "+v"(pv[it][1]));
+        }
+    };
+    auto stem_end = [&](const Coord& c) {
+        const int iy0 = c.ty * TH - 1, ix0 = c.tx * 32 - 1;
+        f4 ssc[2], ssh[2];
+#pragma unroll
+        for (int hq = 0; hq < 2; ++hq) {
+            ssc[hq] = *reinterpret_cast<const f4*>(stp + 320 + oc8 + hq * 4);
+            ssh[hq] = *reinterpret_cast<const f4*>(stp + 352 + oc8 + hq * 4);
+        }
+#pragma unroll
+        for (int it = 0; it < NIT; ++it) {
+            const bool in = ((unsigned)(iy0 + piy[it]) < (unsigned)a.H) & ((unsigned)(ix0 + pix[it]) < (unsigned)a.W);
+#pragma unroll
+            for (int hq = 0; hq < 2; ++hq)
+#pragma unroll
+                for (int r = 0; r < 4; ++r) pv[it][hq][r] = in ? fmaf(fmaxf(pv[it][hq][r], 0.f), ssc[hq][r], ssh[hq][r]) : 0.f;
         }
     };
     auto store_tile = [&]() {
@@ -703,8 +809,19 @@
     }
 
     f4 rsn[MT][NT];
+    float rx[STEM == STEM_RES ? MT : 1][9];
     auto load_res = [&](const Coord& c) {
         const int ty = c.ty, tx = c.tx;
+        if constexpr (STEM == STEM_RES) {
+            const float* __restrict__ sb = a.st_x + (size_t)c.b * a.H * a.W;
+#pragma unroll
+            for (int t = 0; t < MT; ++t) {
+                const int id = wave * MT + t;
+                const int oy = ty * TH + (id >> 1), ox = tx * 32 + (id & 1) * 16 + li;
+                window_load(sb, oy, ox, rx[t]);
+            }
+            return;
+        }
         const size_t rbase = (size_t)c.b * hw * 32;
 #pragma unroll
         for (int t = 0; t < MT; ++t) {
@@ -722,8 +839,21 @@
     cur.tx = t_begin - cur.b * a.tiles - cur.ty * a.tiles_x;
     Coord nxt = cur;
     load_tile(cur);
-    load_res(cur);
+    if (!STEM_PIPE) load_res(cur);
     wait_vmcnt_imm<0>();
+    if constexpr (STEM_PIPE) patch_write(cur);
+    if constexpr (STEM != STEM_NONE) __syncthreads();
+    if constexpr (STEM_PIPE) {
+        stem_begin();
+#pragma unroll
+        for (int t = 0; t < 9; ++t) stem_tap(t);
+        stem_end(cur);
+        Coord n1 = cur;
+        advance(n1);
+        if (t_begin + NWG < t_end) load_tile(n1);
+        wait_lgkmcnt0();
+        wg_barrier();
+    }
     unsigned int ph[6] = {0, 0, 0, 0, 0, 0};
     unsigned long long tk = 0;
     auto stamp = [&](int i) {
@@ -739,6 +869,7 @@
         advance(nxt);
         stamp(-1);
         store_tile();
+        if constexpr (STEM_PIPE) patch_write(nxt);
         stamp(0);
         __syncthreads();
         stamp(1);
@@ -750,11 +881,35 @@
             const int oy = oy0 + (id >> 1), ox = ox0 + (id & 1) * 16 + li;
             pixo[t] = (oy < a.Ho && ox < a.Wo) ? oy * a.Wo + ox : -1;
 #pragma unroll
-            for (int n = 0; n < NT; ++n) rs[t][n] = rsn[t][n];
-        }
-        const bool has_res = a.res != nullptr;
-        if (L + NWG < t_end) load_res(nxt);
-        if (L + NWG < t_end) load_tile(nxt);
+            for (int n = 0; n < NT; ++n) rs[t][n] = STEM_PIPE ? (f4){0.f, 0.f, 0.f, 0.f} : rsn[t][n];
+        }
+        if constexpr (STEM == STEM_RES) {
+#pragma unroll
+            for (int t = 0; t < MT; ++t) {
+                const int id = wave * MT + t;
+                window_pad(oy0 + (id >> 1), ox0 + (id & 1) * 16 + li, rx[t]);
+            }
+#pragma unroll
+            for (int n = 0; n < NT; ++n) {
+                f4 wq[9], sbi, ssc, ssh;
+                stem_consts(n * 16 + kq * 4, wq, sbi, ssc, ssh);
+#pragma unroll
+                for (int t = 0; t < MT; ++t) {
+                    rs[t][n] = stem_quad(rx[t], wq, sbi, ssc, ssh);
+                    asm volatile("" : "+v"(rs[t][n]));
+                }
+            }
+        }
+        const bool has_res = STEM == STEM_RES || (!STEM_PIPE && a.res != nullptr);
+        if (!STEM_PIPE && L + NWG < t_end) load_res(nxt);
+        if constexpr (STEM_PIPE) {
+            Coord n2 = nxt;
+            advance(n2);
+            if (L + 2 * NWG < t_end) load_tile(n2);
+            stem_begin();
+        } else {
+            if (L + NWG < t_end) load_tile(nxt);
+        }
         stamp(2);
 
         f4 acc[MT][NT];
@@ -767,6 +922,7 @@
 #pragma unroll
         for (int tap = 0; tap < 9; ++tap) {
             if (tap < 8) read_frags(fr[(tap + 1) & 1], tap + 1);
+            if constexpr (STEM_PIPE) stem_tap(tap);
             const Frags& f = fr[tap & 1];
 #pragma unroll
             for (int t = 0; t < MT; ++t)
@@ -778,6 +934,14 @@
                     }
                     acc[t][n] = __builtin_amdgcn_mfma_f32_16x16x32_bf16(f.wh[n], f.xh[t], acc[t][n], 0, 0, 0);
                 }
+            if constexpr (STEM_PIPE) {
+                constexpr int NM = MT * NT * (TERMS == 3 ? 3 : 1);
+#pragma unroll
+                for (int i = 0; i < NM; ++i) {
+                    __builtin_amdgcn_sched_group_barrier(0x008, 1, 0);
+                    __builtin_amdgcn_sched_group_barrier(0x002, (32 + NM - 1) / NM, 0);
+                }
+            }
         }
 
         if constexpr (STAMP) {
@@ -787,6 +951,7 @@
                 for (int n = 0; n < NT; ++n) asm volatile("" : "+v"(acc[t][n]));
         }
         stamp(3);
+        if constexpr (STEM_PIPE) stem_end(nxt);
         float* __restrict__ yb = a.y + (size_t)b * hw * 32;
         f4 gsum[NT], gsq[NT];
 #pragma unroll
@@ -870,14 +1035,12 @@
     __syncthreads();
     float* yrow = y + ((size_t)b * H + oy) * W * C + cq * 4;
     for (int ox = px0; ox < W; ox += pstep) {
-        f4 acc = bi;
+        float xv[9];
 #pragma unroll
         for (int kh = 0; kh < 3; ++kh)
 #pragma unroll
-            for (int kw = 0; kw < 3; ++kw) acc += wv[kh * 3 + kw] * rows[kh * WP + ox + kw];
-#pragma unroll
-        for (int r = 0; r < 4; ++r) acc[r] = fmaxf(acc[r], 0.f);
-        *reinterpret_cast<f4*>(yrow + (size_t)ox * C) = acc * sc + sh;
+            for (int kw = 0; kw < 3; ++kw) xv[kh * 3 + kw] = rows[kh * WP + ox + kw];
+        *reinterpret_cast<f4*>(yrow + (size_t)ox * C) = stem_quad(xv, wv, bi, sc, sh);
     }
 }
 
@@ -1130,12 +1293,13 @@
     return on;
 }
 
-template <int TERMS, int TH>
+template <int TERMS, int TH, int STEM = STEM_NONE>
 int launch_conv32_persistent_t(const ConvArgs& a, int batch, const bf8* whi, const bf8* wlo, hipStream_t st) {
     using G = ConvGeom<1, TH>;
     constexpr int NIMG = (TERMS == 3) ? 2 : 1;
-    constexpr size_t LDS_BYTES = sizeof(bf8) * (size_t)(NIMG * 4 * G::PL + NIMG * 9 * 128) + (TH == 4 ? 2 * 4 * 32 * sizeof(float) : 0);
-    auto kern = conv3x3_c32_persistent_kernel<TERMS, TH>;
+    constexpr size_t LDS_BYTES = sizeof(bf8) * (size_t)(NIMG * 4 * G::PL + NIMG * 9 * 128) + (TH == 4 ? 2 * 4 * 32 * sizeof(float) : 0) +
+                                 stem_lds_bytes(STEM);
+    auto kern = conv3x3_c32_persistent_kernel<TERMS, TH, false, STEM>;
     if (int rc = eg_ensure_dynamic_lds(reinterpret_cast<const void*>(kern), LDS_BYTES, "conv3x3 (32 -> 32, persistent)")) return rc;
     const int total = a.tiles * batch;
     const int cap = 512;
@@ -1146,47 +1310,59 @@
     hipLaunchKernelGGL(kern, dim3(grid), dim3(256), LDS_BYTES, st, a, whi, wlo, total, tpw);
     return eg_check_launch("conv3x3 (32 -> 32, persistent)");
 }
-int launch_conv32_persistent(const ConvArgs& a, int batch, int precision, int th, hipStream_t st) {
+template <int STEM>
+int launch_conv32_stamps(const ConvArgs& a, int batch, const bf8* whi, const bf8* wlo, hipStream_t st) {
+    static unsigned int* dbg = nullptr;
+    const int nwords = 512 * 4 * 8;
+    if (!dbg && hipMalloc(&dbg, nwords * sizeof(unsigned int)) != hipSuccess) return EG_ERR_HIP;
+    (void)hipMemsetAsync(dbg, 0, nwords * sizeof(unsigned int), st);
+    ConvArgs b = a;
+    b.dbg = dbg;
+    constexpr size_t LDS_BYTES = sizeof(bf8) * (size_t)(2 * 4 * ConvGeom<1, 4>::PL + 2 * 9 * 128) + 2 * 4 * 32 * sizeof(float) +
+                                 stem_lds_bytes(STEM);
+    auto kern = conv3x3_c32_persistent_kernel<3, 4, true, STEM>;
+    if (int rc = eg_ensure_dynamic_lds(reinterpret_cast<const void*>(kern), LDS_BYTES, "conv3x3 (stamps)")) return rc;
+    const int total = a.tiles * batch;
+    int grid = total < 512 ? total : 512;
+    grid = eg_cdiv(total, eg_cdiv(total, grid));
+    if (grid >= 8) grid = (int)eg_round_up(grid, 8);
+    hipLaunchKernelGGL(kern, dim3(grid), dim3(256), LDS_BYTES, st, b, whi, wlo, total, 0);
+    static unsigned int host[512 * 4 * 8];
+    if (hipMemcpyAsync(host, dbg, sizeof(host), hipMemcpyDeviceToHost, st) != hipSuccess || hipStreamSynchronize(st) != hipSuccess) return EG_ERR_HIP;
+    double sum[6] = {0, 0, 0, 0, 0, 0};
+    int nw = 0;
+    for (int w = 0; w < grid * 4; ++w) {
+        if (host[w * 8 + 3] == 0) continue;
+        ++nw;
+        for (int i = 0; i < 6; ++i) sum[i] += host[w * 8 + i];
+    }
+    const double tiles_per_wave = (double)total / grid;
+    static const char* const stem_name[3] = {"", ", stem input made during the taps", ", stem residual"};
+    fprintf(stderr, "conv32 stamps (cycles per tile and wave, %d waves, %s residual%s): store_tile %.0f  barrier1 %.0f  issue_loads %.0f  taps %.0f  epilogue %.0f  barrier2 %.0f\n",
+            nw, (a.res || STEM == STEM_RES) ? "with" : "no", stem_name[STEM], sum[0] / nw / tiles_per_wave, sum[1] / nw / tiles_per_wave, sum[2] / nw / tiles_per_wave,
+            sum[3] / nw / tiles_per_wave, sum[4] / nw / tiles_per_wave, sum[5] / nw / tiles_per_wave);
+    return eg_check_launch("conv3x3 (32 -> 32, stamps)");
+}
+template <int STEM>
+int launch_conv32_persistent_s(const ConvArgs& a, int batch, int precision, int th, const bf8* whi, const bf8* wlo, hipStream_t st) {
+    static const bool stamp = [] { const char* e = getenv("EG_CONV32_STAMP"); return e && e[0] == '1'; }();
+    if (stamp && precision == EG_PREC_BF16X3 && th == 4) return launch_conv32_stamps<STEM>(a, batch, whi, wlo, st);
+    if constexpr (STEM == STEM_NONE) {
+        if (th == 8) {
+            if (precision == EG_PREC_BF16X3) return launch_conv32_persistent_t<3, 8>(a, batch, whi, wlo, st);
+            return launch_conv32_persistent_t<1, 8>(a, batch, whi, wlo, st);
+        }
+    }
+    if (precision == EG_PREC_BF16X3) return launch_conv32_persistent_t<3, 4, STEM>(a, batch, whi, wlo, st);
+    return launch_conv32_persistent_t<1, 4, STEM>(a, batch, whi, wlo, st);
+}
+int launch_conv32_persistent(const ConvArgs& a, int batch, int precision, int th, hipStream_t st, int stem = STEM_NONE) {
     const size_t f32_floats = (size_t)9 * 32 * 32;
     const bf8* whi = reinterpret_cast<const bf8*>(a.w + f32_floats);
     const bf8* wlo = whi + (size_t)9 * 4 * 32;
-    static const bool stamp = [] { const char* e = getenv("EG_CONV32_STAMP"); return e && e[0] == '1'; }();
-    if (stamp && precision == EG_PREC_BF16X3 && th == 4) {
-        static unsigned int* dbg = nullptr;
-        const int nwords = 512 * 4 * 8;
-        if (!dbg && hipMalloc(&dbg, nwords * sizeof(unsigned int)) != hipSuccess) return EG_ERR_HIP;
-        (void)hipMemsetAsync(dbg, 0, nwords * sizeof(unsigned int), st);
-        ConvArgs b = a;
-        b.dbg = dbg;
-        constexpr size_t LDS_BYTES = sizeof(bf8) * (size_t)(2 * 4 * ConvGeom<1, 4>::PL + 2 * 9 * 128) + 2 * 4 * 32 * sizeof(float);
-        auto kern = conv3x3_c32_persistent_kernel<3, 4, true>;
-        if (int rc = eg_ensure_dynamic_lds(reinterpret_cast<const void*>(kern), LDS_BYTES, "conv3x3 (stamps)")) return rc;
-        const int total = a.tiles * batch;
-        int grid = total < 512 ? total : 512;
-        grid = eg_cdiv(total, eg_cdiv(total, grid));
-        if (grid >= 8) grid = (int)eg_round_up(grid, 8);
-        hipLaunchKernelGGL(kern, dim3(grid), dim3(256), LDS_BYTES, st, b, whi, wlo, total, 0);
-        static unsigned int host[512 * 4 * 8];
-        if (hipMemcpyAsync(host, dbg, sizeof(host), hipMemcpyDeviceToHost, st) != hipSuccess || hipStreamSynchronize(st) != hipSuccess) return EG_ERR_HIP;
-        double sum[6] = {0, 0, 0, 0, 0, 0};
-        int nw = 0;
-        for (int w = 0; w < grid * 4; ++w) {
-            if (host[w * 8 + 3] == 0) continue;
-            ++nw;
-            for (int i = 0; i < 6; ++i) sum[i] += host[w * 8 + i];
-        }
-        const double tiles_per_wave = (double)total / grid;
-        fprintf(stderr, "conv32 stamps (cycles per tile and wave, %d waves, %s residual): store_tile %.0f  barrier1 %.0f  issue_loads %.0f  taps %.0f  epilogue %.0f  barrier2 %.0f\n",
-                nw, a.res ? "with" : "no", sum[0] / nw / tiles_per_wave, sum[1] / nw / tiles_per_wave, sum[2] / nw / tiles_per_wave, sum[3] / nw / tiles_per_wave,
-                sum[4] / nw / tiles_per_wave, sum[5] / nw / tiles_per_wave);
-        return eg_check_launch("conv3x3 (32 -> 32, stamps)");
-    }
-    if (th == 8) {
-        if (precision == EG_PREC_BF16X3) return launch_conv32_persistent_t<3, 8>(a, batch, whi, wlo, st);
-        return launch_conv32_persistent_t<1, 8>(a, batch, whi, wlo, st);
-    }
-    if (precision == EG_PREC_BF16X3) return launch_conv32_persistent_t<3, 4>(a, batch, whi, wlo, st);
-    return launch_conv32_persistent_t<1, 4>(a, batch, whi, wlo, st);
+    if (stem == STEM_IN_PIPE) return launch_conv32_persistent_s<STEM_IN_PIPE>(a, batch, precision, th, whi, wlo, st);
+    if (stem == STEM_RES) return launch_conv32_persistent_s<STEM_RES>(a, batch, precision, th, whi, wlo, st);
+    return launch_conv32_persistent_s<STEM_NONE>(a, batch, precision, th, whi, wlo, st);
 }
 
 int conv_tile_rows(int cin, int cout, int stride) {
@@ -1222,10 +1398,11 @@
 
 namespace {
 struct ShortcutArgs { const float* x; const float* wimg; const float* vec; int h, w, cin, stride; };
+struct StemArgs { const float* spec; const float* w; const float* bias; const float* scale; const float* shift; int mode; };
 int conv3x3_dispatch(const float* x, const float* w, const float* bias, const float* scale, const float* shift, const float* gate, const float* residual,
                      float* y, float* gap_partial, float* gap_sq, int32_t batch, int32_t h, int32_t wdt, int32_t cin, int32_t cout, int32_t stride,
                      int32_t relu, int32_t nchw_out, int32_t precision, void* stream, const float* in_scale = nullptr, const float* in_shift = nullptr,
-                     const uint32_t* res_bits = nullptr, const ShortcutArgs* sc = nullptr);
+                     const uint32_t* res_bits = nullptr, const ShortcutArgs* sc = nullptr, const StemArgs* stem = nullptr);
 }
 extern "C" int eg_conv3x3_se(const float* x, const float* w, const float* bias, const float* scale, const float* shift, const float* gate,
                              const float* residual, float* y, float* gap_partial, int32_t batch, int32_t h, int32_t wdt, int32_t cin,
@@ -1259,13 +1436,14 @@
 int conv3x3_dispatch(const float* x, const float* w, const float* bias, const float* scale, const float* shift, const float* gate, const float* residual,
                      float* y, float* gap_partial, float* gap_sq, int32_t batch, int32_t h, int32_t wdt, int32_t cin, int32_t cout, int32_t stride,
                      int32_t relu, int32_t nchw_out, int32_t precision, void* stream, const float* in_scale, const float* in_shift, const uint32_t* res_bits,
-                     const ShortcutArgs* sc) {
-    EG_REQUIRE(x && w && y && batch > 0 && h > 0 && wdt > 0, EG_ERR_BAD_ARG, "eg_conv3x3: null pointer or empty shape");
+                     const ShortcutArgs* sc, const StemArgs* stem) {
+    const bool stem_in = stem && stem->mode != STEM_RES, stem_res = stem && stem->mode == STEM_RES;
+    EG_REQUIRE((x || stem_in) && w && y && batch > 0 && h > 0 && wdt > 0, EG_ERR_BAD_ARG, "eg_conv3x3: null pointer or empty shape");
     EG_REQUIRE(!res_bits || (residual && !gate && ((size_t)batch * h * wdt * cout) % 32 == 0), EG_ERR_BAD_ARG,
                "eg_conv3x3_res_masked: the bit mask needs a residual, no gate and a map of a multiple of 32 elements");
     EG_REQUIRE((in_scale == nullptr) == (in_shift == nullptr) && (!in_scale || (precision != EG_PREC_F32 && cin % 32 == 0 && eg_aligned16(in_scale) &&
                eg_aligned16(in_shift))), EG_ERR_BAD_ARG, "eg_conv3x3: the input affine needs both vectors, a split-bf16 mode and cin %% 32 == 0");
-    EG_REQUIRE(!gate || residual, EG_ERR_BAD_ARG, "eg_conv3x3_se: a gate needs a residual");
+    EG_REQUIRE(!gate || residual || stem_res, EG_ERR_BAD_ARG, "eg_conv3x3_se: a gate needs a residual");
     EG_REQUIRE(!residual || (!nchw_out && stride == 1 && cout % 4 == 0 && (!gate || eg_aligned16(gate)) && eg_aligned16(residual) && residual != y),
                EG_ERR_BAD_ARG, "eg_conv3x3_se: the fused residual needs NHWC output, stride 1, cout %% 4 == 0 and a residual buffer distinct from y");
     EG_REQUIRE(eg_aligned16(x) && eg_aligned16(w) && eg_aligned16(y), EG_ERR_ALIGN, "eg_conv3x3: pointers must be 16-byte aligned");
@@ -1307,6 +1485,14 @@
         if (split == 4) return launch_conv_split_t<128, 2, 4, 2, 2, 3, 2>(a, batch, whi, wlo, st);
         return launch_conv<128, 8, 1, 4, 2, 2, 2>(a, batch, precision, st);
     }
+    if (stem) {
+        EG_REQUIRE(cin == 32 && cout == 32 && stride == 1 && precision != EG_PREC_F32 && !nchw_out && conv32_persistent_enabled() && th == 4 && !sc && !in_scale &&
+                   !res_bits && !gap_sq && !(stem_in && (x || residual || gate)) && !(stem_res && residual) && (stem->mode == STEM_IN_PIPE || stem_res),
+                   EG_ERR_UNSUPPORTED, "conv3x3: the stem recompute serves the persistent 32 -> 32 kernel with 4-row tiles in the split-bf16 modes");
+        EG_REQUIRE(stem->spec && stem->w && stem->bias && stem->scale && stem->shift, EG_ERR_BAD_ARG, "conv3x3: stem recompute: null pointer");
+        a.st_x = stem->spec; a.st_w = stem->w; a.st_b = stem->bias; a.st_scale = stem->scale; a.st_shift = stem->shift;
+        return launch_conv32_persistent(a, batch, precision, th, st, stem->mode);
+    }
     if (cin == 32 && coutp == 32 && cout == 32 && stride == 1 && precision != EG_PREC_F32 && !nchw_out && conv32_persistent_enabled())
         return launch_conv32_persistent(a, batch, precision, th, st);
     if (cin == 32 && coutp == 32 && stride == 1 && th == 4) return launch_conv<32, 2, 1, 4, 4, 1>(a, batch, precision, st);
@@ -1417,6 +1603,28 @@
                             nullptr, nullptr, nullptr, &sc);
 }
 
+extern "C" int32_t eg_stem_fused_available(int32_t precision) {
+    return precision != EG_PREC_F32 && conv32_persistent_enabled() && conv_tile_rows(32, 32, 1) == 4;
+}
+extern "C" int eg_se_block_fused_stem(const float* spec, const float* stem_w, const float* stem_b, const float* stem_scale, const float* stem_shift,
+                                      const float* stem_map, const float* conv1_w, const float* scale1, const float* shift1, const float* conv2_w,
+                                      const float* scale2, const float* shift2, const float* se_w1, const float* se_b1, const float* se_w2, const float* se_b2,
+                                      float* t1, float* out, float* gap_partial, float* gate, int32_t batch, int32_t h, int32_t wdt, int32_t precision,
+                                      void* stream) {
+    EG_REQUIRE(spec && stem_w && stem_b && stem_scale && stem_shift && conv1_w && scale1 && shift1 && conv2_w && scale2 && shift2 && t1 && out && gap_partial &&
+               gate, EG_ERR_BAD_ARG, "eg_se_block_fused_stem: null pointer");
+    EG_REQUIRE(eg_stem_fused_available(precision), EG_ERR_UNSUPPORTED,
+               "eg_se_block_fused_stem: needs a split-bf16 mode and the persistent 32 -> 32 kernel with 4-row tiles");
+    const StemArgs in{spec, stem_w, stem_b, stem_scale, stem_shift, STEM_IN_PIPE}, res{spec, stem_w, stem_b, stem_scale, stem_shift, STEM_RES};
+    if (int rc = conv3x3_dispatch(nullptr, conv1_w, nullptr, scale1, shift1, nullptr, nullptr, t1, gap_partial, nullptr, batch, h, wdt, 32, 32, 1, 1, 0, precision,
+                                  stream, nullptr, nullptr, nullptr, nullptr, &in)) return rc;
+    const int tiles1 = eg_conv3x3_gap_tiles(h, wdt, 32, 32, 1);
+    if (int rc = se_gate_pre_launch(t1, gap_partial, tiles1, conv2_w, scale2, shift2, se_w1, se_b1, se_w2, se_b2, gate, batch, h, wdt, 32, stream, nullptr,
+                                    nullptr, nullptr)) return rc;
+    return conv3x3_dispatch(t1, conv2_w, nullptr, scale2, shift2, gate, stem_map, out, nullptr, nullptr, batch, h, wdt, 32, 32, 1, 0, 0, precision, stream, nullptr,
+                            nullptr, nullptr, nullptr, stem_map ? nullptr : &res);
+}
+
 extern "C" int eg_se_residual_relu(const float* y, const float* gate, const float* x_in, const float* ds_w,
                                    const float* ds_scale, const float* ds_shift, float* out, int32_t batch, int32_t ho,
                                    int32_t wo, int32_t c, int32_t h_in, int32_t w_in, int32_t cin, int32_t stride, void* stream) {
diff --git a/emotiongestures_amd/csrc/generator.hip b/emotiongestures_amd/csrc/generator.hip
--- a/emotiongestures_amd/csrc/generator.hip
+++ b/emotiongestures_amd/csrc/generator.hip
@@ -285,6 +285,7 @@
     int64_t txt_fc1_w, txt_fc1_b;
     int Cpad;
     bool keep_taps = false;
+    bool stem_fused = true, stem_res = true;
     bool concurrent = false;
     mutable hipStream_t side[2] = {nullptr, nullptr};
     mutable hipEvent_t ev_fork = nullptr, ev_join[2] = {nullptr, nullptr};
@@ -461,8 +462,12 @@
     float* bufs[3] = {P(ws, w.act[0]), P(ws, w.act[1]), P(ws, w.act[2])};
     float *gap = P(ws, w.gap), *gate = P(ws, w.gate);
     int xi = 0, h = g->H1, wd = g->W1, bi = 0;
-    EG_TRY(eg_stem_conv(spec, arena + g->stem_w, arena + g->stem_b, arena + g->stem_scale, arena + g->stem_shift, bufs[0], B, g->H1,
-                        g->W1, 32, st));
+    const BlockW& b0 = g->blocks[0];
+    const bool stem_fused = g->stem_fused && g->fuse_se && !g->keep_taps && !b0.ds && b0.cin == 32 && b0.cout == 32 && b0.stride == 1 &&
+                            eg_stem_fused_available(prec);
+    if (!stem_fused || !g->stem_res)
+        EG_TRY(eg_stem_conv(spec, arena + g->stem_w, arena + g->stem_b, arena + g->stem_scale, arena + g->stem_shift, bufs[0], B, g->H1,
+                            g->W1, 32, st));
     if (g->keep_taps)
         EG_HIP_TRY(hipMemcpyAsync(P(ws, w.tap_stem), bufs[0], sizeof(float) * (size_t)B * g->H1 * g->W1 * 32, hipMemcpyDeviceToDevice, st), "tap copy");
     for (int s = 0; s < 3; ++s) {
@@ -470,6 +475,14 @@
             const BlockW& bw = g->blocks[bi];
             const int t1 = (xi + 1) % 3, t2 = (xi + 2) % 3;
             const int ho = (h + 2 - 3) / bw.stride + 1, wo = (wd + 2 - 3) / bw.stride + 1;
+            if (stem_fused && bi == 0) {
+                EG_TRY(eg_se_block_fused_stem(spec, arena + g->stem_w, arena + g->stem_b, arena + g->stem_scale, arena + g->stem_shift,
+                                              g->stem_res ? nullptr : bufs[xi], arena + bw.c1.w, arena + bw.c1.scale, arena + bw.c1.shift, arena + bw.c2.w,
+                                              arena + bw.c2.scale, arena + bw.c2.shift, arena + bw.se_w1, arena + bw.se_b1, arena + bw.se_w2, arena + bw.se_b2,
+                                              bufs[t1], bufs[t2], gap, gate, B, h, wd, prec, st));
+                xi = t2;
+                continue;
+            }
             if (g->fuse_se && (!bw.ds || prec != EG_PREC_F32)) {
                 EG_TRY(eg_se_block_fused(bufs[xi], arena + bw.c1.w, arena + bw.c1.scale, arena + bw.c1.shift, arena + bw.c2.w, arena + bw.c2.scale,
                                          arena + bw.c2.shift, arena + bw.se_w1, arena + bw.se_b1, arena + bw.se_w2, arena + bw.se_b2,
@@ -695,6 +708,8 @@
     g->fold = cfg->reserved[2] != 0;
     g->fuse_se = cfg->reserved[3] == 0;
     g->shared_chip = cfg->reserved[4] != 0;
+    if (const char* e = getenv("EG_STEM_FUSED")) g->stem_fused = e[0] != '0';
+    if (const char* e = getenv("EG_STEM_RES")) g->stem_res = e[0] != '0';
     const EgGeneratorConfig& c = g->cfg;
     g->H1 = c.n_mels; g->W1 = c.spec_len;
     g->H2 = (g->H1 - 1) / 2 + 1; g->W2 = (g->W1 - 1) / 2 + 1;
diff --git a/emotiongestures_amd/ops.py b/emotiongestures_amd/ops.py
--- a/emotiongestures_amd/ops.py
+++ b/emotiongestures_amd/ops.py
@@ -113,7 +113,8 @@
     return out
 
 
-def se_block_fused(x_nhwc, c1, c2, se_w1, se_b1, se_w2, se_b2, cout, stride=1, ds_weight=None, ds_scale=None, ds_shift=None, precision="bf16x3"):
+def se_block_fused(x_nhwc, c1, c2, se_w1, se_b1, se_w2, se_b2, cout, stride=1, ds_weight=None, ds_scale=None, ds_shift=None, precision="bf16x3",
+                   return_parts=False):
     lib = L.load()
     x = _need_cuda(x_nhwc, "x")
     dev = x.device
@@ -131,7 +132,29 @@
                                   _ptr(_need_cuda(se_b1, "b1")), _ptr(_need_cuda(se_w2, "w2")), _ptr(_need_cuda(se_b2, "b2")), _ptr(dsw), _ptr(ds_scale),
                                   _ptr(ds_shift), _ptr(t1), _ptr(out), _ptr(gap), _ptr(gate), _ptr(scv), B, H, W, Cin, cout, stride,
                                   L.precision_code(precision), _stream(dev)), "eg_se_block_fused")
-    return out
+    return (out, t1, gap, gate) if return_parts else out
+
+
+def stem_fused_available(precision="bf16x3"):
+    return bool(L.load().eg_stem_fused_available(L.precision_code(precision)))
+
+
+def se_block_fused_stem(spec, stem_weight, stem_bias, stem_scale, stem_shift, c1, c2, se_w1, se_b1, se_w2, se_b2, precision="bf16x3", stem_map=None,
+                        return_parts=False):
+    lib = L.load()
+    x = _need_cuda(spec, "spec")
+    dev = x.device
+    B, H, W = x.shape
+    w9 = stem_weight.detach().reshape(32, 9).t().contiguous().to(dev, torch.float32)
+    tiles = lib.eg_conv3x3_gap_tiles(H, W, 32, 32, 1)
+    t1, out = torch.empty(B, H, W, 32, device=dev), torch.empty(B, H, W, 32, device=dev)
+    gap, gate = torch.empty(B, tiles, 32, device=dev), torch.empty(B, 32, device=dev)
+    L.check(lib.eg_se_block_fused_stem(_ptr(x), _ptr(w9), _ptr(_need_cuda(stem_bias, "bias")), _ptr(_need_cuda(stem_scale, "scale")),
+                                       _ptr(_need_cuda(stem_shift, "shift")), _ptr(stem_map), _ptr(c1[0]), _ptr(c1[2]), _ptr(c1[3]), _ptr(c2[0]),
+                                       _ptr(c2[2]), _ptr(c2[3]), _ptr(_need_cuda(se_w1, "w1")), _ptr(_need_cuda(se_b1, "b1")),
+                                       _ptr(_need_cuda(se_w2, "w2")), _ptr(_need_cuda(se_b2, "b2")), _ptr(t1), _ptr(out), _ptr(gap), _ptr(gate), B, H, W,
+                                       L.precision_code(precision), _stream(dev)), "eg_se_block_fused_stem")
+    return (out, t1, gap, gate) if return_parts else out
 
 
 def linear(x, weight, bias=None, res1=None, res2=None, relu=False, a_shift=0, a_seq=0, precision="f32", packed=None):
diff --git a/include/emogest.h b/include/emogest.h
--- a/include/emogest.h
+++ b/include/emogest.h
@@ -327,6 +327,11 @@
                       const float* shift2, const float* se_w1, const float* se_b1, const float* se_w2, const float* se_b2, const float* ds_w,
                       const float* ds_scale, const float* ds_shift, float* t1, float* out, float* gap_partial, float* gate, float* sc_vec,
                       int32_t batch, int32_t h, int32_t wdt, int32_t cin, int32_t cout, int32_t stride, int32_t precision, void* stream);
+int32_t eg_stem_fused_available(int32_t precision);
+int eg_se_block_fused_stem(const float* spec, const float* stem_w, const float* stem_b, const float* stem_scale, const float* stem_shift,
+                           const float* stem_map, const float* conv1_w, const float* scale1, const float* shift1, const float* conv2_w, const float* scale2,
+                           const float* shift2, const float* se_w1, const float* se_b1, const float* se_w2, const float* se_b2, float* t1, float* out,
+                           float* gap_partial, float* gate, int32_t batch, int32_t h, int32_t wdt, int32_t precision, void* stream);
 int64_t eg_conv3x3_packed_floats(int32_t cin, int32_t cout_pad);
 
 int eg_stem_conv(const float* x, const float* w9xc, const float* bias, const float* scale, const float* shift,
```

Result: no change. 26610 clips/s (-0.2%).
